# william-dawson/NTPoly

Hardware: AMD Instinct MI355X
Metric: TRS2 iters/s + SpGEMM nnz-out/s, N=262k ~200 nnz/row, 1/2/4/8 GPU (higher is better)
Workload: dtype f64

## Files before the change

### include/ntpoly_amd.h

```cpp
#ifndef NTPOLY_AMD_H
#define NTPOLY_AMD_H
#include "ntpoly_amd_process_grid.h"
#include "ntpoly_amd_psmatrix.h"
#include "ntpoly_amd_smatrix.h"
#include "ntpoly_amd_triplet_list.h"
#include "ntpoly_amd_permutation.h"
#include "ntpoly_amd_memory_pool.h"
#include "ntpoly_amd_solver_parameters.h"
#include "ntpoly_amd_density_matrix_solvers.h"
#include "ntpoly_amd_sign_solvers.h"
#include "ntpoly_amd_inverse_solvers.h"
#include "ntpoly_amd_square_root_solvers.h"
#include "ntpoly_amd_load_balancer.h"
#include "ntpoly_amd_eigen_bounds.h"
#include "ntpoly_amd_logging.h"
#include "ntpoly_amd_polynomial_solvers.h"
#include "ntpoly_amd_function_solvers.h"
#include "ntpoly_amd_linear_solvers.h"
#include "ntpoly_amd_eigen_solvers.h"
#include "ntpoly_amd_geometry.h"
#ifdef __cplusplus
extern "C" {
#endif

void ntpoly_amd_allreduce_max(double* values, const int* n);
int ntpoly_amd_band_order(const int* ih, int* newpos, long long* bandwidth);
void ntpoly_amd_band_scope_counts(long long* out);
void ntpoly_amd_band_searches(long long* out);
void ntpoly_amd_barrier();
void ntpoly_amd_block_algebra_counts(long long* out);
int ntpoly_amd_block_order(const int* ih, int* position);
int ntpoly_amd_block_order_of_pattern(const int* ih, int* position, int* ns);
void ntpoly_amd_block_scope_counts(long long* out);
void ntpoly_amd_column_fused_counts(long long* out);
int ntpoly_amd_comm_rank();
int ntpoly_amd_comm_size();
void ntpoly_amd_comm_split_matrix(const int* ih_this, int* ih_split, int* my_color, bool* split_slice);
void ntpoly_amd_complex_fusion_counts(long long* out);
int ntpoly_amd_device_count();
void ntpoly_amd_drop_block_caches();
void ntpoly_amd_exchange_stats(long long* out);
void ntpoly_amd_fill_prepartitioned(const int* ih_this, const int* ih_triplet_list);
void ntpoly_amd_finalize_comm();
void ntpoly_amd_fusion_counts(long long* out);
void ntpoly_amd_gather_matrix_to_process(const int* ih_this, int* ih_local, const int* within_slice_id);
int ntpoly_amd_get_option(const char* name);
void ntpoly_amd_get_spgemm_accum(long long* out, double* dout);
void ntpoly_amd_get_unique_id(char* out128);
void ntpoly_amd_grid_comm_info(const int* ih_grid, int* out);
void ntpoly_amd_halo_segment(const int* dim, const int* nranks, const int* s, const int* kmin, const int* kmax, int* a, int* b);
void ntpoly_amd_increment_identity(const int* ih_identity, int* ih_matB, const double* alpha);
void ntpoly_amd_init_comm(const char* id128, const int* rank, const int* nranks);
void ntpoly_amd_last_block_stats(long long* out, double* fill);
void ntpoly_amd_last_grouped_stats(long long* out, double* ratio);
void ntpoly_amd_last_spgemm_stats(long long* out, float* ms_numeric, float* ms_total);
int ntpoly_amd_last_spgemm_thin();
void ntpoly_amd_log_element_bool(const char* key, const int* nk, const bool* v);
void ntpoly_amd_log_element_int(const char* key, const int* nk, const int* v);
void ntpoly_amd_log_element_real(const char* key, const int* nk, const double* v);
void ntpoly_amd_log_element_string(const char* key, const int* nk, const char* v, const int* nv);
void ntpoly_amd_log_enter();
void ntpoly_amd_log_exit();
void ntpoly_amd_log_header(const char* text, const int* n);
void ntpoly_amd_log_list_element(const char* key, const int* nk);
void ntpoly_amd_malloc_stats(long long* calls, double* ms);
int ntpoly_amd_matrix_is_complex(const int* ih_this);
void ntpoly_amd_matrix_local_columns(const int* ih_this, int* c0, int* c1);
void ntpoly_amd_memory(long long* in_use, long long* cached);
int ntpoly_amd_norm_axpby(const int* ih_matA, const int* ih_matB, const double* alpha, const double* beta, double* norm);
void ntpoly_amd_panel_exchange_layout(const int* dim, const int* nranks, const int* me, const long long* req, const long long* cnt, int* sa, int* sb, long long* soff, int* ra, int* rb, long long* zoff);
void ntpoly_amd_panel_product_counts(long long* out);
void ntpoly_amd_panel_range(const int* dim, const int* nranks, const int* rank, int* c0, int* c1);
void ntpoly_amd_permutation_set(int* ih_this, const int* n, const int* index_lookup);
int ntpoly_amd_recurrence_step(const int* ih_P, const int* ih_Tkm2, int* ih_Tk, int* ih_R, const double* a, const double* c);
void ntpoly_amd_recurrence_step_count(long long* out);
void ntpoly_amd_release_cache();
void ntpoly_amd_reset_spgemm_accum();
void ntpoly_amd_session_begin(const int* complex_ok);
void ntpoly_amd_session_end();
void ntpoly_amd_set_option(const char* name, const int* value);
void ntpoly_amd_slab_algebra_counts(long long* out);
void ntpoly_amd_split_process_grid(const int* ih_old_grid, int* ih_new_grid, int* my_color, bool* split_slice);
void ntpoly_amd_square_root_order(const int* ih_Input, int* ih_Output, const int* ih_solver_parameters, const int* inverse, const int* order);
void ntpoly_amd_synchronize();
void ntpoly_amd_thin_slab_counts(long long* out);
void ntpoly_amd_tile2_counts(long long* out);
void ntpoly_amd_trace_get(double* value, double* energy, double* sigma, long long* nnz);
int ntpoly_amd_trace_iterations();
void ntpoly_amd_trace_times(double* setup_ms, double* loop_ms);
void ntpoly_amd_triplets_get(const int* ih_list, int* col, int* row, double* val);
void ntpoly_amd_triplets_set_c(int* ih_list, const long long* n, const int* col, const int* row, const double* val_ri);
void ntpoly_amd_triplets_set_r(int* ih_list, const long long* n, const int* col, const int* row, const double* val);
void ntpoly_amd_trs2_step(int* ih_X, int* ih_X2, const int* ih_WH, const double* trace, const double* threshold, double* energy_out, double* sigma_out, double* trace_io);

#ifdef __cplusplus
}
#endif
#endif
```

### ntpoly_amd/csrc/common.cpp

```cpp
#include <cstdio>
#include <cstdlib>
#include <chrono>
#include "common.hpp"

#include <cstring>
#include <mutex>

namespace ntp {

void fatal(const char* file, int line, const std::string& msg) {
  std::fprintf(stderr, "[ntpoly_amd] FATAL %s:%d: %s\n", file, line, msg.c_str());
  std::fflush(stderr);
  std::abort();
}

Context& ctx() {
  static Context* c = new Context();
  return *c;
}

void ensure_init() {
  Context& c = ctx();
  if (c.initialised) return;
  int ndev = 0;
  hipError_t e = hipGetDeviceCount(&ndev);
  if (e != hipSuccess || ndev == 0)
    NTP_FATAL("no HIP device visible: the ntpoly_amd engine has no CPU fallback");
  int local_rank = 0;
  if (const char* lr = std::getenv("LOCAL_RANK")) local_rank = std::atoi(lr);
  c.device = local_rank % ndev;
  HIP_CHECK(hipSetDevice(c.device));
  HIP_CHECK(hipStreamCreateWithFlags(&c.stream, hipStreamNonBlocking));
  HIP_CHECK(hipStreamCreateWithFlags(&c.comm_stream, hipStreamNonBlocking));
  hipDeviceProp_t prop;
  HIP_CHECK(hipGetDeviceProperties(&prop, c.device));
  c.num_cus = prop.multiProcessorCount;
  c.initialised = true;
}

long long& host_sync_count() {
  static long long n = 0;
  return n;
}
namespace {
struct SyncClock {
  bool on = std::getenv("NTPOLY_AMD_DEBUG_SYNC") != nullptr;
  long long calls = 0, slow = 0;
  double ms = 0.0;
  ~SyncClock() {
    if (on) std::fprintf(stderr, "[sync_stream] %lld waits, %.1f ms in them, %lld longer than 10 ms\n", calls, ms, slow);
  }
};
SyncClock& sync_clock() {
  static SyncClock c;
  return c;
}
}
void sync_stream() {
  host_sync_count() += 1;
  SyncClock& c = sync_clock();
  if (!c.on) {
    HIP_CHECK(hipStreamSynchronize(ctx().stream));
    return;
  }
  const auto t0 = std::chrono::steady_clock::now();
  HIP_CHECK(hipStreamSynchronize(ctx().stream));
  const double ms = std::chrono::duration<double, std::milli>(std::chrono::steady_clock::now() - t0).count();
  c.calls += 1;
  c.ms += ms;
  c.slow += ms > 10.0 ? 1 : 0;
}

namespace {
struct Pool {
  std::mutex mu;
  std::map<size_t, std::vector<void*>> free_lists;
  std::map<void*, size_t> live;
  std::map<const void*, unsigned long long> serial_of;
  unsigned long long next_serial = 1;
  size_t in_use = 0, cached = 0;
  long long n_malloc = 0;
  double ms_malloc = 0.0;
};
Pool& pool() {
  static Pool* p = new Pool();
  return *p;
}
size_t bucket(size_t bytes) {
  if (bytes < 512) return 512;
  const size_t big = (size_t)64 << 20;
  if (bytes > big) {
    const size_t want = bytes + bytes / 8;
    size_t p2 = big;
    while (p2 * 2 <= want) p2 <<= 1;
    const size_t step = p2 / 4;
    return (want + step - 1) / step * step;
  }
  size_t b = 512;
  while (b < bytes) b <<= 1;
  return b;
}
}

void* dev_alloc(size_t bytes) {
  ensure_init();
  const size_t b = bucket(bytes);
  Pool& P = pool();
  std::lock_guard<std::mutex> g(P.mu);
  auto it = P.free_lists.find(b);
  void* p = nullptr;
  size_t got = b;
  if (it == P.free_lists.end() || it->second.empty()) {
    it = P.free_lists.end();
    if (b >= ((size_t)1 << 20))
      for (auto jt = P.free_lists.upper_bound(b); jt != P.free_lists.end() && jt->first <= 2 * b; ++jt)
        if (!jt->second.empty()) { it = jt; got = jt->first; break; }
  }
  if (it != P.free_lists.end() && !it->second.empty()) {
    p = it->second.back();
    it->second.pop_back();
    P.cached -= got;
  } else {
    const auto t0 = std::chrono::steady_clock::now();
    hipError_t e = hipMalloc(&p, b);
    if (e != hipSuccess) {
      (void)hipGetLastError();
      for (auto& kv : P.free_lists) {
        for (void* q : kv.second) (void)hipFree(q);
        kv.second.clear();
      }
      P.cached = 0;
      HIP_CHECK(hipMalloc(&p, b));
    }
    P.n_malloc += 1;
    const double ms = std::chrono::duration<double, std::milli>(std::chrono::steady_clock::now() - t0).count();
    P.ms_malloc += ms;
    static const bool dbg = std::getenv("NTPOLY_AMD_DEBUG_ALLOC") != nullptr;
    if (dbg)
      std::fprintf(stderr, "[dev_alloc] hipMalloc %.1f MB (asked %.1f MB) took %.1f ms%s; in use %.1f GB, cached %.1f GB\n", b / 1048576.0,
                   bytes / 1048576.0, ms, e != hipSuccess ? " AFTER releasing the cache (out of memory)" : "", P.in_use / 1073741824.0,
                   P.cached / 1073741824.0);
  }
  P.live[p] = got;
  P.serial_of[p] = P.next_serial++;
  P.in_use += got;
  return p;
}

void dev_free(void* p) {
  if (!p) return;
  Pool& P = pool();
  std::lock_guard<std::mutex> g(P.mu);
  auto it = P.live.find(p);
// ... 96 lines not shown
```

### ntpoly_amd/csrc/common.hpp

```cpp
#pragma once
#include <hip/hip_runtime.h>

#include <cstdint>
#include <cstdio>
#include <cstdlib>
#include <map>
#include <string>
#include <utility>
#include <memory>
#include <vector>

namespace ntp {

[[noreturn]] void fatal(const char* file, int line, const std::string& msg);
#define NTP_FATAL(msg) ::ntp::fatal(__FILE__, __LINE__, (msg))
#define HIP_CHECK(expr)                                                              \
  do {                                                                               \
    hipError_t e_ = (expr);                                                          \
    if (e_ != hipSuccess)                                                            \
      ::ntp::fatal(__FILE__, __LINE__, std::string(#expr) + ": " + hipGetErrorString(e_)); \
  } while (0)

struct Context {
  int device = 0;
  hipStream_t stream = nullptr;
  hipStream_t comm_stream = nullptr;
  int num_cus = 256;
  bool initialised = false;
};
Context& ctx();
void ensure_init();
inline hipStream_t stream() { return ctx().stream; }
void sync_stream();
long long& host_sync_count();

struct ScalarFetch {
  const void* src[16];
  int words[16];
  void* dst[16];
  int n = 0;
  void add(const void* dev, int words8, void* host_dst) {
    src[n] = dev; words[n] = words8; dst[n] = host_dst; ++n;
  }
  void run();
};

void* dev_alloc(size_t bytes);
void dev_free(void* p);
unsigned long long dev_alloc_serial(const void* p);
void dev_release_cache();
size_t dev_bytes_in_use();
size_t dev_bytes_cached();
void dev_malloc_stats(long long* calls, double* ms);

template <typename T>
struct DevBuf {
  T* p = nullptr;
  size_t n = 0;
  DevBuf() = default;
  explicit DevBuf(size_t count) { alloc(count); }
  DevBuf(const DevBuf&) = delete;
  DevBuf& operator=(const DevBuf&) = delete;
  DevBuf(DevBuf&& o) noexcept : p(o.p), n(o.n) { o.p = nullptr; o.n = 0; }
  DevBuf& operator=(DevBuf&& o) noexcept {
    if (this != &o) {
      release();
      p = o.p; n = o.n; o.p = nullptr; o.n = 0;
    }
    return *this;
  }
  ~DevBuf() { release(); }
  void alloc(size_t count) {
    release();
    n = count;
    p = static_cast<T*>(dev_alloc((count ? count : 1) * sizeof(T)));
  }
  void release() {
    if (p) dev_free(p);
    p = nullptr; n = 0;
  }
  void upload(const T* host, size_t count) {
    if (count) HIP_CHECK(hipMemcpyAsync(p, host, count * sizeof(T), hipMemcpyHostToDevice, stream()));
  }
  void download(T* host, size_t count) const {
    const size_t bytes = count * sizeof(T);
    if (bytes > 0 && bytes <= 1024 && bytes % 8 == 0) {
      ScalarFetch f;
      f.add(p, (int)(bytes / 8), host);
      f.run();
      return;
    }
    if (count) HIP_CHECK(hipMemcpyAsync(host, p, bytes, hipMemcpyDeviceToHost, stream()));
    sync_stream();
  }
  void zero() { if (n) HIP_CHECK(hipMemsetAsync(p, 0, n * sizeof(T), stream())); }
};

constexpr size_t kIndexSlack = 1024;

struct SlabPlan {
  DevBuf<int32_t> blk_lo, blk_w, blk_kmin, blk_kn;
  DevBuf<int64_t> blk_toff;
  int64_t total = 0;
  int max_w = 0, max_kn = 0;
  int align = 0;
};
struct SlabForm {
  DevBuf<int32_t> first, last, count;
  DevBuf<int64_t> off;
  DevBuf<int64_t> tile_off;
  DevBuf<double> val, tiles;
  int64_t slots = 0;
  bool no_tile2 = false;
  std::unique_ptr<SlabPlan> next_plan;
  std::shared_ptr<struct DevMat> origin;
  mutable int64_t span_sum = -1;
  int row_pad = 1;
  DevBuf<int32_t> lab, plast;
  bool labelled() const { return lab.p != nullptr; }
};

struct DevMat {
  int32_t rows = 0, cols = 0;
  bool cplx = false;
  int64_t nnz = 0;
  DevBuf<int64_t> outer;
  DevBuf<int32_t> inner;
  DevBuf<double> val;
  DevBuf<int32_t> cnt;
  int64_t slots = 0;
  bool loose() const { return cnt.p != nullptr; }
  mutable int zero_free = 0;
  std::unique_ptr<SlabForm> slab;
  bool expanded() const { return slab != nullptr; }
  std::shared_ptr<struct BlockForm> blk;
  bool blocked() const { return blk != nullptr; }
  mutable int block_hint = 0;
  mutable int slab_hint = 0;

  DevMat() = default;
  DevMat(int32_t r, int32_t c, bool z) { reset_empty(r, c, z); }
  DevMat(DevMat&&) noexcept = default;
  DevMat& operator=(DevMat&&) noexcept = default;
  void reset_empty(int32_t r, int32_t c, bool z);
  void alloc(int32_t r, int32_t c, bool z, int64_t nz);
  DevMat clone() const;
  size_t wval() const { return cplx ? 2 : 1; }
};

DevMat packed_copy(const DevMat& M);

struct HostTriplets {
  std::vector<int32_t> col, row;
  std::vector<double> val;
  bool cplx = false;
  size_t size() const { return col.size(); }
};

}
```

### ntpoly_amd/csrc/kernels.hip

```cpp
#include "kernels.hpp"
#include "device_util.hpp"
#include "spgemm_grouped.hpp"
#include "slab_types.hpp"
#include "spgemm_tile.hpp"
#include "spgemm_block.hpp"

#include <hip/hip_runtime.h>

#include <algorithm>
#include <cstdlib>
#include <climits>
#include <cmath>
#include <cstring>
#include <type_traits>
#include <numeric>
#include <utility>

#include <rocprim/device/device_radix_sort.hpp>

namespace ntp {

namespace {

__global__ __launch_bounds__(1024) void k_scan_excl_i64(const int64_t* __restrict__ in,
// ... 533 lines not shown
        }
      }
      if (!more) break;
      s_cur = s_nxt;
      use_a = !use_a;
    }
    asm volatile("s_waitcnt vmcnt(0)" ::: "memory");
    kv0 = nk0; kv1 = nk1;
    bv0 = nb0; bv1 = nb1;
  }
  __builtin_amdgcn_wave_barrier();

#pragma unroll
  for (int r = 0; r < 2; ++r) {
    const bool act = r == 0 ? act0 : act1;
    if (!act) continue;
    const int j = r == 0 ? j0 : j1;
    const int lo = r == 0 ? lo0 : lo1, span = r == 0 ? span0 : span1;
    const double* acc = r == 0 ? acc0 : acc1;
    const int64_t base = tmpoff[j];
    int cnt = 0;
    for (int s0 = 0; s0 < span; s0 += WAVE) {
      const int s = s0 + lane;
      const double v = (s < span) ? acc[s] : 0.0;
      const double sv = __dmul_rn(alpha, v);
      const bool keep = (s < span) && ((dense_rule & 1) ? (fabs(v) > threshold) : (fabs(sv) > threshold));
      const unsigned long long m = __ballot(keep);
      if (keep) {
        const int64_t pos = base + cnt + __popcll(m & lanemask_lt());
        out_inner[pos] = lo + s;
        out_val[pos] = sv;
      }
      cnt += __popcll(m);
    }
    if (lane == 0) count[j] = cnt;
  }
}

template <typename T>
__global__ __launch_bounds__(256) void k_slab_expand_a(Csc A, const int32_t* __restrict__ afirst,
                                                       const int64_t* __restrict__ aeoff, T* __restrict__ aexp) {
  const int k = (blockIdx.x * blockDim.x + threadIdx.x) / WAVE;
  if (k >= A.cols) return;
  const int lane = lane_id();
  const int64_t s = A.outer[k], e = A.outer[k + 1];
  if (e <= s) return;
  const T* __restrict__ Av = static_cast<const T*>(A.val);
  T* __restrict__ dst = aexp + aeoff[k] - afirst[k];
  for (int64_t p = s + lane; p < e; p += WAVE) {
    const int r = A.inner[p];
    const int prev = (p > s) ? A.inner[p - 1] : r - 1;
    dst[r] = Av[p];
    for (int h = prev + 1; h < r; ++h) dst[h] = Sc<T>::zero();
  }
}

__global__ void k_span_aligned(const int32_t* __restrict__ cmin, const int32_t* __restrict__ cmax, int32_t* __restrict__ span, int n, int al) {
  const int k = blockIdx.x * blockDim.x + threadIdx.x;
  if (k >= n) return;
  const int f = cmin[k], l = cmax[k];
  span[k] = l >= f ? (l / al + 1) * al - f / al * al : 0;
}
template <typename T>
__global__ __launch_bounds__(256) void k_aligned_offsets(const int32_t* __restrict__ cmin, const int32_t* __restrict__ cmax,
                                                         int64_t* __restrict__ off, T* __restrict__ exp, int n, int al) {
  const int k = (blockIdx.x * blockDim.x + threadIdx.x) / WAVE;
  if (k >= n) return;
  const int lane = lane_id();
  const int f = cmin[k], l = cmax[k];
  if (l < f) return;
  const int64_t slot = off[k];
  const int head = f - f / al * al, tail = (l / al + 1) * al - 1 - l;
  for (int i = lane; i < head; i += WAVE) exp[slot + i] = Sc<T>::zero();
  for (int i = lane; i < tail; i += WAVE) exp[slot + head + (l - f + 1) + i] = Sc<T>::zero();
  if (lane == 0) off[k] = slot + head;
}

template <int J>
__global__ __launch_bounds__(256) void k_slab_plan(int ncols, const int32_t* __restrict__ bfirst,
                                                   const int32_t* __restrict__ blast, const int32_t* __restrict__ cmin,
                                                   const int32_t* __restrict__ cmax, int32_t* __restrict__ blk_lo,
                                                   int32_t* __restrict__ blk_w, int32_t* __restrict__ blk_kmin,
                                                   int32_t* __restrict__ blk_kn, int64_t* __restrict__ bsz,
                                                   int64_t* __restrict__ tsz, int nblocks, int align16 = 0) {
  const int b = (blockIdx.x * blockDim.x + threadIdx.x) / WAVE;
  const int lane = lane_id();
  if (b < nblocks) {
    const int j = b * J + lane;
    const bool has = lane < J && j < ncols && blast[min(j, ncols - 1)] >= 0;
    const int kmin = wave_min_i32(has ? bfirst[j] : INT_MAX), kmax = wave_max_i32(has ? blast[j] : -1);
    if (kmax >= kmin && kmax - kmin >= 4096) {
      if (lane == 0) {
        blk_lo[b] = 0;
        blk_w[b] = 1 << 30;
        blk_kmin[b] = kmin;
        blk_kn[b] = kmax - kmin + 1;
        bsz[b] = 0;
        tsz[b] = 0;
      }
    } else {
      int lo = INT_MAX, hi = -1;
      for (int k = (kmax >= kmin) ? kmin + lane : 0; k <= kmax; k += WAVE) {
        const int c0 = cmin[k], c1 = cmax[k];
        if (c1 >= c0) {
          lo = min(lo, c0);
          hi = max(hi, c1 + 1);
        }
      }
      lo = wave_min_i32(lo);
      hi = wave_max_i32(hi);
      if (lane == 0) {
        if (align16 > 0 && hi > lo) {
          lo = lo / align16 * align16;
          hi = (hi + align16 - 1) / align16 * align16;
        }
        const int w = (hi > lo) ? hi - lo : 0;
        const int kn = (w > 0 && kmax >= kmin) ? kmax - kmin + 1 : 0;
        blk_lo[b] = w > 0 ? lo : 0;
        blk_w[b] = w;
        blk_kmin[b] = kn > 0 ? kmin : 0;
        blk_kn[b] = kn;
        bsz[b] = (int64_t)((kn + 1) & ~1) * J;
        tsz[b] = (int64_t)w * J;
      }
    }
  }
}

constexpr int kOffParts = 64;
__global__ __launch_bounds__(256) void k_slab_offsets(const int32_t* __restrict__ blk_w, const int32_t* __restrict__ blk_kn,
                                                      const int64_t* __restrict__ tsz, const int64_t* __restrict__ bsz,
                                                      int nblocks, int part, int64_t* __restrict__ toff,
                                                      int64_t* __restrict__ boff, unsigned long long* __restrict__ stats) {
  __shared__ long long wsum[2][4];
  __shared__ int wmax[2][4];
  const int lane = lane_id(), wave = threadIdx.x / WAVE;
  const int p0 = blockIdx.x * part, p1 = min(nblocks, p0 + part);
  if (p0 >= nblocks) return;
  auto block_sum = [&](long long& a, long long& b) {
    a = wave_sum_i64(a);
    b = wave_sum_i64(b);
    __syncthreads();
    if (lane == 0) { wsum[0][wave] = a; wsum[1][wave] = b; }
    __syncthreads();
    a = wsum[0][0] + wsum[0][1] + wsum[0][2] + wsum[0][3];
    b = wsum[1][0] + wsum[1][1] + wsum[1][2] + wsum[1][3];
  };
  long long carry_t = 0, carry_b = 0;
  {
    int i = threadIdx.x;
    for (; i + 7 * 256 < p0; i += 8 * 256) {
      long long t[8], u[8];
#pragma unroll
      for (int e = 0; e < 8; ++e) {
        t[e] = tsz[i + e * 256];
        u[e] = boff ? (long long)bsz[i + e * 256] : 0;
      }
#pragma unroll
      for (int e = 0; e < 8; ++e) { carry_t += t[e]; carry_b += u[e]; }
    }
    for (; i < p0; i += 256) {
      carry_t += tsz[i];
      if (boff) carry_b += bsz[i];
    }
  }
  block_sum(carry_t, carry_b);
  int mw = 0, mk = 0;
  for (int base = p0; base < p1; base += 256) {
    const int i = base + threadIdx.x;
    const long long t = i < p1 ? (long long)tsz[i] : 0, b = (boff && i < p1) ? (long long)bsz[i] : 0;
    if (i < p1) {
      mw = max(mw, blk_w[i]);
      mk = max(mk, blk_kn[i]);
    }
    long long xt = t, xb = b;
    for (int o = 1; o < WAVE; o <<= 1) {
      const long long at = __shfl_up(xt, o, WAVE), ab = __shfl_up(xb, o, WAVE);
      if (lane >= o) { xt += at; xb += ab; }
    }
    __syncthreads();
    if (lane == WAVE - 1) { wsum[0][wave] = xt; wsum[1][wave] = xb; }
    __syncthreads();
    long long pt = carry_t + xt - t, pb = carry_b + xb - b;
    for (int q = 0; q < wave; ++q) { pt += wsum[0][q]; pb += wsum[1][q]; }
    if (i < p1) {
      toff[i] = pt;
      if (boff) boff[i] = pb;
    }
    carry_t += wsum[0][0] + wsum[0][1] + wsum[0][2] + wsum[0][3];
    carry_b += wsum[1][0] + wsum[1][1] + wsum[1][2] + wsum[1][3];
  }
  if (p1 == nblocks && threadIdx.x == 0) {
    toff[nblocks] = carry_t;
    if (boff) boff[nblocks] = carry_b;
  }
  mw = wave_max_i32(mw);
  mk = wave_max_i32(mk);
  __syncthreads();
  if (lane == 0) { wmax[0][wave] = mw; wmax[1][wave] = mk; }
  __syncthreads();
  if (threadIdx.x == 0 && stats) {
    atomicMax(&stats[16], (unsigned long long)max(max(wmax[0][0], wmax[0][1]), max(wmax[0][2], wmax[0][3])));
    atomicMax(&stats[17], (unsigned long long)max(max(wmax[1][0], wmax[1][1]), max(wmax[1][2], wmax[1][3])));
  }
}

template <typename T, int J>
__global__ __launch_bounds__(256) void k_slab_expand_b(Csc B, const int32_t* __restrict__ blk_kmin,
                                                       const int32_t* __restrict__ blk_kn,
                                                       const int64_t* __restrict__ blk_boff, T* __restrict__ bblk,
                                                       int nblocks, int pitch, int fuse_a,
                                                       const int64_t* __restrict__ aeoff, T* __restrict__ aexp,
                                                       const int32_t* __restrict__ clen,
                                                       int64_t* __restrict__ blk_prod) {
  extern __shared__ __attribute__((aligned(16))) char smem[];
  T* tile = reinterpret_cast<T*>(smem);
  const int b = xcd_block(nblocks);
  if (b < 0) return;
  const int kn = blk_kn[b], kmin = blk_kmin[b];
  if (kn == 0 && !fuse_a) return;
  const bool tiled = kn > 0;
  const T* __restrict__ Bv = static_cast<const T*>(B.val);
  const int wave = threadIdx.x / WAVE, lane = lane_id();
  constexpr int CH = 5, NCOL = J / 4;
  int idx[NCOL][CH];
  T val[NCOL][CH];
#pragma unroll
  for (int q = 0; q < NCOL; ++q) {
    const int j = min(b * J + wave + 4 * q, B.cols - 1);
    const int64_t s = B.outer[j];
#pragma unroll
    for (int c = 0; c < CH; ++c) {
      idx[q][c] = B.inner[s + c * WAVE + lane];
      val[q][c] = Bv[s + c * WAVE + lane];
    }
  }
  const int kne = (kn + 1) & ~1;
  for (int jj = 0; jj < J; ++jj)
    for (int i = threadIdx.x; i < kne; i += blockDim.x) tile[jj * pitch + i] = Sc<T>::zero();
  __syncthreads();
  long long nprod = 0;
#pragma unroll
  for (int q = 0; q < NCOL; ++q) {
    const int jj = wave + 4 * q;
    const int j = b * J + jj;
    if (j >= B.cols) break;
    const int64_t s = B.outer[j], e = col_end(B, j);
    if (e <= s) continue;
    const int first = readlane_i32(idx[q][0], 0);
    T* __restrict__ dst = fuse_a ? aexp + aeoff[j] - first : nullptr;
    int carry = first - 1;
#pragma unroll
    for (int c = 0; c < CH; ++c) {
      const int64_t p = s + c * WAVE + lane;
      const int r = idx[q][c];
      int prev = __shfl_up(r, 1, WAVE);
      if (lane == 0) prev = carry;
      if (p < e) {
        if (clen) nprod += clen[r];
        if (tiled) tile[jj * pitch + (r - kmin)] = val[q][c];
        if (fuse_a) {
          dst[r] = val[q][c];
          for (int h = prev + 1; h < r; ++h) dst[h] = Sc<T>::zero();
        }
      }
      carry = readlane_i32(r, WAVE - 1);
    }
    for (int64_t p = s + CH * WAVE + lane; p < e; p += WAVE) {
      const int r = B.inner[p];
      const T v = Bv[p];
      if (clen) nprod += clen[r];
      if (tiled) tile[jj * pitch + (r - kmin)] = v;
      if (fuse_a) {
        const int prev = B.inner[p - 1];
        dst[r] = v;
        for (int h = prev + 1; h < r; ++h) dst[h] = Sc<T>::zero();
      }
    }
  }
  nprod = wave_sum_i64(nprod);
  __shared__ long long sprod[4];
  if (lane == 0) sprod[wave] = nprod;
  __syncthreads();
  if (threadIdx.x == 0) blk_prod[b] = sprod[0] + sprod[1] + sprod[2] + sprod[3];
  T* __restrict__ out = bblk + blk_boff[b];
  const int total = kne * J;
// ... 1548 lines not shown
__global__ void k_remap_gather(const unsigned long long* __restrict__ keys, const unsigned int* __restrict__ payload,
                               int64_t nkeep, const T* __restrict__ val, int32_t* __restrict__ inner_out,
                               T* __restrict__ val_out, int32_t* __restrict__ colcount) {
  const int64_t p = (int64_t)blockIdx.x * blockDim.x + threadIdx.x;
  const bool live = p < nkeep;
  const unsigned long long k = live ? keys[p] : ~0ull;
  if (live) {
    inner_out[p] = (int32_t)(k & 0xffffffffull);
    val_out[p] = val[payload[p]];
  }
  const int col = (int)(k >> 32), lane = lane_id();
  const int prev = __shfl_up(col, 1, WAVE);
  const bool leader = live && (lane == 0 || col != prev);
  const unsigned long long heads = __ballot(leader), alive = __ballot(live);
  if (leader) {
    const unsigned long long later = heads & ~((2ull << lane) - 1ull);
    const int end = later ? __builtin_ctzll(later) : (int)__popcll(alive);
    atomicAdd(&colcount[col], end - lane);
  }
}
__global__ void k_count_valid(const unsigned long long* __restrict__ keys, int64_t n,
                              unsigned long long* __restrict__ out) {
  __shared__ unsigned long long sc[4];
  unsigned long long c = 0;
  for (int64_t p = (int64_t)blockIdx.x * blockDim.x + threadIdx.x; p < n; p += (int64_t)gridDim.x * blockDim.x)
    c += keys[p] != ~0ull ? 1ull : 0ull;
  c = (unsigned long long)wave_sum_i64((int64_t)c);
  if (lane_id() == 0) sc[threadIdx.x / WAVE] = c;
  __syncthreads();
  if (threadIdx.x == 0) atomicAdd(out, sc[0] + sc[1] + sc[2] + sc[3]);
}

__global__ void k_shift_outer(const int64_t* __restrict__ in, int64_t* __restrict__ out, int n, int64_t shift) {
  const int j = blockIdx.x * blockDim.x + threadIdx.x;
  if (j <= n) out[j] = in[j] + shift;
}

__global__ void k_rebase_i64(const int64_t* __restrict__ in, int64_t* __restrict__ out, int n, int64_t add) {
  const int i = blockIdx.x * blockDim.x + threadIdx.x;
  if (i < n) out[i] = in[i] - in[0] + add;
}
__global__ void k_linear_i64(int64_t* __restrict__ out, int64_t n, int64_t step) {
  const int64_t i = (int64_t)blockIdx.x * blockDim.x + threadIdx.x;
  if (i < n) out[i] = i * step;
}
__global__ void k_fill_i64(int64_t* __restrict__ out, int64_t n, int64_t v) {
  const int64_t i = (int64_t)blockIdx.x * blockDim.x + threadIdx.x;
  if (i < n) out[i] = v;
}
__global__ void k_row_range(Csc A, int* __restrict__ mm) {
  const int j = blockIdx.x * blockDim.x + threadIdx.x;
  int lo = INT_MAX, hi = -1;
  if (j < A.cols) {
    const int64_t s = A.outer[j], e = A.outer[j + 1];
    if (e > s) {
      lo = A.inner[s];
      hi = A.inner[e - 1];
    }
  }
  lo = wave_min_i32(lo);
  hi = wave_max_i32(hi);
  if (lane_id() == 0) {
    if (lo != INT_MAX) atomicMin(&mm[0], lo);
    if (hi >= 0) atomicMax(&mm[1], hi);
  }
}

}

EngineOptions& options() {
  static EngineOptions* o = [] {
    auto* e = new EngineOptions();
    if (const char* v = std::getenv("NTPOLY_AMD_HALO_OVERLAP")) e->halo_overlap = std::atoi(v);
    if (const char* v = std::getenv("NTPOLY_AMD_SPGEMM_FMA")) e->spgemm_fma = std::atoi(v);
    if (const char* v = std::getenv("NTPOLY_AMD_ARITHMETIC")) {
      const std::string a(v);
      if (a == "fma") e->spgemm_fma = 1;
      else if (a == "unfused") e->spgemm_fma = 0;
      else NTP_FATAL("NTPOLY_AMD_ARITHMETIC must be fma or unfused, not " + a);
    }
    if (const char* v = std::getenv("NTPOLY_AMD_TILE_ROWS")) e->tile_rows = std::atoi(v);
    if (const char* v = std::getenv("NTPOLY_AMD_TILE_WAVES")) e->tile_waves = std::atoi(v);
    if (const char* v = std::getenv("NTPOLY_AMD_PLAN_AHEAD")) e->plan_ahead = std::atoi(v);
    if (const char* v = std::getenv("NTPOLY_AMD_SLAB_ALGEBRA")) e->slab_algebra = std::atoi(v);
    if (const char* v = std::getenv("NTPOLY_AMD_PANEL_SESSIONS")) e->panel_sessions = std::atoi(v);
    if (const char* v = std::getenv("NTPOLY_AMD_COMPLEX_PANELS")) e->complex_panels = std::atoi(v);
    if (const char* v = std::getenv("NTPOLY_AMD_THIN_SLAB_COMPLEX")) e->thin_slab_complex = std::atoi(v);
    if (const char* v = std::getenv("NTPOLY_AMD_COMPLEX_POLY_SESSIONS")) e->complex_poly_sessions = std::atoi(v);
    if (const char* v = std::getenv("NTPOLY_AMD_COMPLEX_DENSITY")) e->complex_density = std::atoi(v);
    if (const char* v = std::getenv("NTPOLY_AMD_BLOCK_SCOPE_COMPLEX")) e->block_scope_complex = std::atoi(v);
    if (const char* v = std::getenv("NTPOLY_AMD_BLOCK_UNFUSED")) e->block_unfused = std::atoi(v);
    return e;
  }();
  return *o;
}
SpgemmStats& last_spgemm_stats() {
  static SpgemmStats* s = new SpgemmStats();
  return *s;
}
SpgemmAccum& spgemm_accum() {
  static SpgemmAccum* a = new SpgemmAccum();
  return *a;
}

namespace {
template <typename TIn>
void scan_async(const TIn* d_in, int64_t* d_out, int64_t n) {
  if (n <= 4096) {
    if constexpr (sizeof(TIn) == 8) hipLaunchKernelGGL(k_scan_excl_i64, dim3(1), dim3(1024), 0, stream(), (const int64_t*)d_in, d_out, n);
    else hipLaunchKernelGGL(k_scan_excl_i32, dim3(1), dim3(1024), 0, stream(), (const int32_t*)d_in, d_out, n);
    return;
  }
  const int nb = (int)((n + 2047) / 2048);
  DevBuf<int64_t> sums((size_t)nb), offs((size_t)nb + 1);
  hipLaunchKernelGGL((k_scan_block_sums<TIn>), dim3(nb), dim3(256), 0, stream(), d_in, n, sums.p);
  hipLaunchKernelGGL(k_scan_excl_i64, dim3(1), dim3(1024), 0, stream(), sums.p, offs.p, (int64_t)nb);
  hipLaunchKernelGGL((k_scan_block_apply<TIn>), dim3(nb), dim3(256), 0, stream(), d_in, n, offs.p, d_out);
}
void reduce_sum2_async(const double* part, int n, double* out_dev) {
  if (n <= 8192) {
    hipLaunchKernelGGL(k_reduce_sum2, dim3(1), dim3(256), 0, stream(), part, n, out_dev, n);
    return;
  }
  const int chunk = 2048, g = (n + chunk - 1) / chunk;
  DevBuf<double> lvl((size_t)2 * g);
  hipLaunchKernelGGL(k_reduce_sum2, dim3(g), dim3(256), 0, stream(), part, n, lvl.p, chunk);
  hipLaunchKernelGGL(k_reduce_sum2, dim3(1), dim3(256), 0, stream(), lvl.p, g, out_dev, g);
}
}

constexpr int FT_BLOCKS = 64;
__global__ __launch_bounds__(256) void k_fused_totals(const int32_t* __restrict__ count, int n, const long long* __restrict__ a,
                                                      const long long* __restrict__ b, const double* __restrict__ part,
                                                      int m, const double* __restrict__ lvl_in, double* __restrict__ out,
                                                      int stage) {
  __shared__ long long si[3][4];
  __shared__ double sd[2][4];
  const int wave = threadIdx.x / WAVE, lane = lane_id();
  long long c = 0, x = 0, y = 0;
  double d = 0.0, t = 0.0;
  if (stage == 0) {
    const int g = blockIdx.x;
    const int n0 = (int)((int64_t)n * g / FT_BLOCKS), n1 = (int)((int64_t)n * (g + 1) / FT_BLOCKS);
#pragma unroll 8
    for (int i = n0 + threadIdx.x; i < n1; i += 256) c += count[i];
    const int m0 = (int)((int64_t)m * g / FT_BLOCKS), m1 = (int)((int64_t)m * (g + 1) / FT_BLOCKS);
#pragma unroll 2
    for (int i = m0 + threadIdx.x; i < m1; i += 256) {
      x += a[i];
      if (b) y += b[i];
      d = __dadd_rn(d, part[2 * i]);
      t = __dadd_rn(t, part[2 * i + 1]);
    }
  } else {
    const long long* li = reinterpret_cast<const long long*>(lvl_in);
    for (int g = threadIdx.x; g < FT_BLOCKS; g += 256) {
      c += li[5 * g]; x += li[5 * g + 1]; y += li[5 * g + 2];
      d = __dadd_rn(d, lvl_in[5 * g + 3]);
      t = __dadd_rn(t, lvl_in[5 * g + 4]);
    }
  }
  c = wave_sum_i64(c); x = wave_sum_i64(x); y = wave_sum_i64(y);
  d = wave_sum_f64(d); t = wave_sum_f64(t);
  if (lane == 0) { si[0][wave] = c; si[1][wave] = x; si[2][wave] = y; sd[0][wave] = d; sd[1][wave] = t; }
  __syncthreads();
  if (threadIdx.x == 0) {
    long long* oi = reinterpret_cast<long long*>(out) + (stage == 0 ? 5 * blockIdx.x : 0);
    double* od = out + (stage == 0 ? 5 * blockIdx.x : 0);
    for (int q = 0; q < 3; ++q) oi[q] = si[q][0] + si[q][1] + si[q][2] + si[q][3];
    od[3] = __dadd_rn(__dadd_rn(sd[0][0], sd[0][1]), __dadd_rn(sd[0][2], sd[0][3]));
    od[4] = __dadd_rn(__dadd_rn(sd[1][0], sd[1][1]), __dadd_rn(sd[1][2], sd[1][3]));
  }
}

void scan_i32_async(const int32_t* d_in, int64_t* d_out, int64_t n) { scan_async<int32_t>(d_in, d_out, n); }
void scan_i64_async(const int64_t* d_in, int64_t* d_out, int64_t n) { scan_async<int64_t>(d_in, d_out, n); }

namespace {
struct FetchArgs {
  const unsigned long long* src[16];
  int words[16];
  int n;
};
__global__ __launch_bounds__(64) void k_fetch(FetchArgs a, unsigned long long* __restrict__ host_mapped) {
  int off = 0;
  for (int s = 0; s < a.n; ++s) {
    for (int i = threadIdx.x; i < a.words[s]; i += 64) host_mapped[off + i] = a.src[s][i];
    off += a.words[s];
  }
  __threadfence_system();
}
}

void ScalarFetch::run() {
  static unsigned long long* host = nullptr;
  static unsigned long long* dev = nullptr;
  constexpr int kMaxWords = 512;
  if (!host) {
    HIP_CHECK(hipHostMalloc(reinterpret_cast<void**>(&host), kMaxWords * 8, hipHostMallocMapped));
    HIP_CHECK(hipHostGetDevicePointer(reinterpret_cast<void**>(&dev), host, 0));
  }
  FetchArgs a;
  a.n = n;
  int total = 0;
  for (int s = 0; s < n; ++s) {
    a.src[s] = static_cast<const unsigned long long*>(src[s]);
    a.words[s] = words[s];
    total += words[s];
  }
  if (total > kMaxWords) NTP_FATAL("ScalarFetch: too many words");
  if (total) hipLaunchKernelGGL(k_fetch, dim3(1), dim3(64), 0, stream(), a, dev);
  sync_stream();
  int off = 0;
  for (int s = 0; s < n; ++s) {
    std::memcpy(dst[s], host + off, (size_t)words[s] * 8);
    off += words[s];
  }
  n = 0;
}

static int64_t exclusive_scan_i64_from_i32(const int32_t* d_in, int64_t* d_out, int64_t n) {
  scan_async<int32_t>(d_in, d_out, n);
  int64_t total = 0;
  ScalarFetch f;
  f.add(d_out + n, 1, &total);
  f.run();
  return total;
}
int64_t exclusive_scan_i64(const int64_t* d_in, int64_t* d_out, int64_t n) {
  scan_async<int64_t>(d_in, d_out, n);
  int64_t total = 0;
  HIP_CHECK(hipMemcpyAsync(&total, d_out + n, sizeof(int64_t), hipMemcpyDeviceToHost, stream()));
  sync_stream();
  return total;
}

namespace {
struct TimedCall {
  hipEvent_t ev[4];
};
std::vector<hipEvent_t>& event_pool() {
  static auto* p = new std::vector<hipEvent_t>();
  return *p;
}
std::vector<TimedCall>& pending_timings() {
  static auto* p = new std::vector<TimedCall>();
  return *p;
}
hipEvent_t get_event() {
  auto& pool = event_pool();
  if (!pool.empty()) {
    hipEvent_t e = pool.back();
    pool.pop_back();
    return e;
// ... 30 lines not shown
  unsigned long long serial = 0, epoch = 0;
  int64_t nnz = -1;
  int32_t cols = 0;
  DevBuf<int32_t> dmin, dmax;
  DevBuf<int64_t> doff;
  DevBuf<double> dexp;
  int64_t max_tile = 0;
  int align = 1;
};
__global__ __launch_bounds__(256) void k_count_zero_values(Csc A, unsigned long long* __restrict__ out) {
  const int j = (blockIdx.x * blockDim.x + threadIdx.x) / WAVE;
  if (j >= A.cols) return;
  const int lane = lane_id();
  const double* __restrict__ v = static_cast<const double*>(A.val);
  int c = 0;
  for (int64_t p = A.outer[j] + lane, e = col_end(A, j); p < e; p += WAVE) c += v[p] == 0.0 ? 1 : 0;
  const unsigned long long m = __ballot(c != 0);
  if (m && lane == 0) atomicAdd(out, 1ull);
}
__global__ void k_span_block_max(const int32_t* __restrict__ span, int n, int J, unsigned long long* __restrict__ out) {
  const int b = blockIdx.x * blockDim.x + threadIdx.x;
  if (b * J >= n) return;
  unsigned long long t = 0;
  for (int j = b * J; j < min(n, (b + 1) * J); ++j) t += (unsigned long long)span[j];
  atomicMax(out, t);
}
DotOperand*& dot_operand_slot() {
  static DotOperand* c = new DotOperand();
  return c;
}
void drop_dot_operand() { *dot_operand_slot() = DotOperand(); }
const DotOperand& dot_operand(const DevMat& D) {
  DotOperand* c = dot_operand_slot();
  const unsigned long long ser = dev_alloc_serial(D.val.p);
  const int want_al = options().spgemm_fma == 1 ? tile_expand_align() : 1;
  if (c->val == D.val.p && c->serial == ser && ser != 0 && c->epoch == value_epoch() && c->nnz == D.nnz && c->cols == D.cols &&
      c->align == want_al)
    return *c;
  const int n = D.cols;
  c->dmin.alloc((size_t)n); c->dmax.alloc((size_t)n); c->doff.alloc((size_t)n + 1);
  DevBuf<int32_t> dlen((size_t)n), dspan((size_t)n);
  hipLaunchKernelGGL(k_col_extent, dim3(cdiv(n, 256)), dim3(256), 0, stream(), view(D), c->dmin.p, c->dmax.p, dlen.p);
  const int al = options().spgemm_fma == 1 ? tile_expand_align() : 1;
  if (al > 1) hipLaunchKernelGGL(k_span_aligned, dim3(cdiv(n, 256)), dim3(256), 0, stream(), c->dmin.p, c->dmax.p, dspan.p, n, al);
  else hipLaunchKernelGGL(k_span_of, dim3(cdiv(n, 256)), dim3(256), 0, stream(), c->dmin.p, c->dmax.p, dspan.p, n);
  scan_async<int32_t>(dspan.p, c->doff.p, (int64_t)n);
  DevBuf<unsigned long long> tmax(1);
  tmax.zero();
  hipLaunchKernelGGL(k_span_block_max, dim3(cdiv(cdiv(n, SLAB_J), 256)), dim3(256), 0, stream(), dspan.p, n, SLAB_J, tmax.p);
  int64_t total = 0;
  unsigned long long hmax = 0;
  {
    ScalarFetch f;
    f.add(c->doff.p + n, 1, &total);
    f.add(tmax.p, 1, &hmax);
    f.run();
  }
  c->max_tile = (int64_t)hmax;
  c->dexp.alloc((size_t)total + 1);
  if (al > 1)
    hipLaunchKernelGGL(k_aligned_offsets<double>, dim3(cdiv((int64_t)n * WAVE, 256)), dim3(256), 0, stream(), c->dmin.p, c->dmax.p,
                       c->doff.p, c->dexp.p, n, al);
  c->align = al;
  hipLaunchKernelGGL(k_slab_expand_a<double>, dim3(cdiv((int64_t)n * WAVE, 256)), dim3(256), 0, stream(), view(D), c->dmin.p,
                     c->doff.p, c->dexp.p);
  c->val = D.val.p;
  c->serial = ser;
  c->epoch = value_epoch();
  c->nnz = D.nnz;
  c->cols = n;
  return *c;
}
}

long long* fusion_counts() {
  static long long c[3] = {0, 0, 0};
  return c;
}
long long* complex_fusion_counts() {
  static long long c[3] = {0, 0, 0};
  return c;
}
long long* tile2_counts() {
  static long long c[2] = {0, 0};
  return c;
}

void flush_spgemm_timers() {
  auto& pend = pending_timings();
  if (pend.empty()) return;
  SpgemmAccum& acc = spgemm_accum();
  for (size_t i = 0; i < pend.size(); ++i) {
    float t_all = 0.f, t_num = 0.f;
    HIP_CHECK(hipEventSynchronize(pend[i].ev[1]));
    HIP_CHECK(hipEventElapsedTime(&t_all, pend[i].ev[0], pend[i].ev[1]));
    HIP_CHECK(hipEventElapsedTime(&t_num, pend[i].ev[2], pend[i].ev[3]));
    acc.ms_total += t_all;
    acc.ms_numeric += t_num;
    if (i + 1 == pend.size()) {
      last_spgemm_stats().ms_total = t_all;
      last_spgemm_stats().ms_numeric = t_num;
    }
    for (int k = 0; k < 4; ++k) event_pool().push_back(pend[i].ev[k]);
  }
  pend.clear();
}

namespace {
__global__ __launch_bounds__(256) void k_pack_slab(int ncols, const int32_t* __restrict__ first, const int32_t* __restrict__ last,
                                                   const int64_t* __restrict__ off, const double* __restrict__ val,
                                                   const int64_t* __restrict__ outer, int32_t* __restrict__ inner,
                                                   double* __restrict__ out) {
  const int j = (blockIdx.x * blockDim.x + threadIdx.x) / WAVE;
  if (j >= ncols) return;
  const int lane = lane_id();
  const int f = first[j], l = last[j];
  int64_t pos = outer[j];
  const double* __restrict__ src = val + off[j];
  for (int r0 = f; r0 <= l; r0 += WAVE) {
    const int r = r0 + lane;
    const double v = r <= l ? src[r - f] : 0.0;
    const unsigned long long m = __ballot(v != 0.0);
    if (v != 0.0) {
      const int64_t q = pos + __popcll(m & lanemask_lt());
      inner[q] = r;
      out[q] = v;
    }
    pos += __popcll(m);
  }
}
__global__ __launch_bounds__(256) void k_pack_slab_c(int ncols, const int32_t* __restrict__ first, const int32_t* __restrict__ last,
                                                     const int64_t* __restrict__ off, const double2* __restrict__ val,
                                                     const int64_t* __restrict__ outer, int32_t* __restrict__ inner,
                                                     double2* __restrict__ out) {
  const int j = (blockIdx.x * blockDim.x + threadIdx.x) / WAVE;
  if (j >= ncols) return;
  const int lane = lane_id();
  const int f = first[j], l = last[j];
  int64_t pos = outer[j];
  const double2* __restrict__ src = val + off[j];
  for (int r0 = f; r0 <= l; r0 += WAVE) {
    const int r = r0 + lane;
    const double2 v = r <= l ? src[r - f] : make_double2(0.0, 0.0);
    const bool nz = v.x != 0.0 || v.y != 0.0;
    const unsigned long long m = __ballot(nz);
    if (nz) {
      const int64_t q = pos + __popcll(m & lanemask_lt());
      inner[q] = r;
      out[q] = v;
    }
    pos += __popcll(m);
  }
}
template <int MAXCH, int NW>
void launch_pair3(int bin_lo, int bin_hi, int wrt, const DevMat& A, const DevMat& B, const int32_t* lo, const int32_t* span,
                  const uint8_t* binarr, const int64_t* tmpoff, int32_t* out_inner, double* out_val, int32_t* count,
                  double alpha, double thr, int dense_rule) {
  const int ngroups = cdiv(B.cols, 2);
  const int nblocks = cdiv(ngroups, NW);
  const size_t lds = (size_t)NW * 2 * (size_t)wrt * sizeof(double);
  hipLaunchKernelGGL((k_spgemm_pair3<MAXCH, NW>), dim3(xcd_grid(nblocks)), dim3(NW * WAVE), lds, stream(), view(A), view(B),
                     lo, span, binarr, bin_lo, bin_hi, tmpoff, out_inner, out_val, count, alpha, thr, dense_rule, nblocks, wrt);
}

template <typename T, int W, int NW>
void launch_window(int bin, const DevMat& A, const DevMat& B, const int32_t* lo, const int32_t* span,
// ... 1059 lines not shown

namespace {
__global__ void k_pack_reduce4(const double* __restrict__ tot, const int* __restrict__ flag, double* __restrict__ out) {
  out[0] = tot[3];
  out[1] = 0.0;
  out[2] = tot[4];
  out[3] = flag[0] == 0 ? 1.0 : 0.0;
}
__global__ void k_slab_runs_addr(const int32_t* __restrict__ first, const int32_t* __restrict__ last,
                                 const unsigned long long* __restrict__ addr, unsigned long long fallback,
                                 SlabRun* __restrict__ runs, int n, int elem_bytes) {
  const int k = blockIdx.x * blockDim.x + threadIdx.x;
  if (k >= n + 4) return;
  const bool any = k < n && last[k] >= first[k];
  SlabRun r;
  const unsigned long long a = any ? addr[k] : fallback;
  r.addr_lo = (uint32_t)a;
  r.addr_hi = (uint32_t)(a >> 32) & 0xffffu;
  r.nbytes = any ? (uint32_t)(last[k] - first[k] + 1) * (uint32_t)elem_bytes : 0u;
  r.flags = kBufferFlags;
  r.first = any ? first[k] : (1 << 30);
  r.first8 = any ? first[k] * elem_bytes : 0;
  r.span62 = any ? (last[k] - first[k] + 1) + 62 : 0;
  r.pad = 0;
  runs[k] = r;
}

__global__ __launch_bounds__(256) void k_slab_order_steps(const int32_t* __restrict__ lab, const int32_t* __restrict__ blk_kmin,
                                                          const int32_t* __restrict__ blk_kn, const int64_t* __restrict__ tile_off,
                                                          const double* __restrict__ tiles_in, const SlabRun* __restrict__ runs,
                                                          int ncols, double* __restrict__ tiles_out, SlabRun* __restrict__ blkruns,
                                                          int32_t* __restrict__ steps, int nblocks) {
  extern __shared__ unsigned long long sk[];
  const int b = xcd_block(nblocks);
  if (b < 0) return;
  const int kn = blk_kn[b], kmin = blk_kmin[b];
  if (kn == 0) return;
  int m = 1;
  while (m < kn) m <<= 1;
  for (int i = threadIdx.x; i < m; i += blockDim.x)
    sk[i] = i < kn ? (((unsigned long long)(unsigned)lab[kmin + i] << 32) | (unsigned)i) : ~0ull;
  __syncthreads();
  for (int k = 2; k <= m; k <<= 1) {
    for (int j = k >> 1; j > 0; j >>= 1) {
      for (int i = threadIdx.x; i < m; i += blockDim.x) {
        const int l = i ^ j;
        if (l > i) {
          const bool up = (i & k) == 0;
          const unsigned long long x = sk[i], y = sk[l];
          if ((x > y) == up) { sk[i] = y; sk[l] = x; }
        }
      }
      __syncthreads();
    }
  }
  const int64_t toff = tile_off[b];
  const int64_t rbase = toff / SLAB_J + 4 * (int64_t)b;
  for (int t = threadIdx.x; t < kn + 4; t += blockDim.x) {
    if (t < kn) {
      const int i = (int)(unsigned)(sk[t] & 0xffffffffull);
      const int k = kmin + i;
      if (steps) steps[rbase + t] = k;
      SlabRun r = runs[k];
      r.pad = i * (int)(SLAB_J * sizeof(double));
      blkruns[rbase + t] = r;
    } else {
      if (steps) steps[rbase + t] = ncols;
      blkruns[rbase + t] = runs[ncols];
    }
  }
  if (!tiles_out) return;
  const double2* __restrict__ src = reinterpret_cast<const double2*>(tiles_in + toff);
  double2* __restrict__ dst = reinterpret_cast<double2*>(tiles_out + toff);
  for (int i = threadIdx.x; i < kn * (SLAB_J / 2); i += blockDim.x) {
    const int t = i / (SLAB_J / 2), q = i % (SLAB_J / 2);
    dst[(size_t)t * (SLAB_J / 2) + q] = src[(size_t)(unsigned)(sk[t] & 0xffffffffull) * (SLAB_J / 2) + q];
  }
}
}

namespace {
template <int J = SLAB_J>
void launch_slab_plan(SlabPlan& P, int n, const int32_t* first, const int32_t* last, const int32_t* afirst, const int32_t* alast,
                      int align, unsigned long long* stats, DevBuf<int64_t>* tile_offsets = nullptr) {
  const int snb = cdiv(n, J);
  P.blk_lo.alloc(snb); P.blk_w.alloc(snb); P.blk_kmin.alloc(snb); P.blk_kn.alloc(snb);
  P.blk_toff.alloc((size_t)snb + 1);
  P.align = align;
  DevBuf<int64_t> bsz(snb), tsz(snb);
  if (tile_offsets) tile_offsets->alloc((size_t)snb + 1);
  hipLaunchKernelGGL((k_slab_plan<J>), dim3(cdiv((int64_t)snb * WAVE, 256)), dim3(256), 0, stream(), n, first, last, afirst,
                     alast, P.blk_lo.p, P.blk_w.p, P.blk_kmin.p, P.blk_kn.p, bsz.p, tsz.p, snb, align);
  if (options().plan_fused != 0) {
    const int part = cdiv(cdiv(snb, kOffParts), 256) * 256;
    hipLaunchKernelGGL(k_slab_offsets, dim3(cdiv(snb, part)), dim3(256), 0, stream(), P.blk_w.p, P.blk_kn.p, tsz.p, bsz.p, snb, part,
                       P.blk_toff.p, tile_offsets ? tile_offsets->p : (int64_t*)nullptr, stats);
    return;
  }
  hipLaunchKernelGGL(k_slab_reduce, dim3(64), dim3(256), 0, stream(), P.blk_w.p, P.blk_kn.p, snb, (const int32_t*)nullptr, 0, stats);
  scan_async<int64_t>(tsz.p, P.blk_toff.p, (int64_t)snb);
  if (tile_offsets) scan_async<int64_t>(bsz.p, tile_offsets->p, (int64_t)snb);
}
}

bool slab_step(DevMat& X, SlabFusion& fu, double threshold, bool dense_rule, const SlabHalo* halo) {
  fu.done = false;
  if (!X.expanded() || X.cplx || (!halo && X.rows != X.cols) || !fu.D || fu.D->cplx || fu.D->loose() || fu.D->expanded() ||
      fu.D->rows != X.rows || fu.D->cols != X.cols || (fu.mode != 1 && fu.mode != 2))
    return false;
  const bool tile = options().spgemm_fma == 1;
  if ((options().spgemm_variant >= 0 && !(tile && options().spgemm_variant / 100 == 6)) || (options().spgemm_fma && !tile) || options().spgemm_force_bin > 0 || !options().fused_update)
    return false;
  const SlabForm& in = *X.slab;
  int trows = 1;
  if (tile) {
    trows = tile_rows();
    while (trows > 1 && (in.row_pad % (16 * trows) != 0 || (halo && halo->row_pad % (16 * trows) != 0))) trows >>= 1;
  }
  const int n = X.cols, snb = cdiv(n, SLAB_J);
  const DotOperand& dop = dot_operand(*fu.D);
  if (!tile && dop.max_tile > SLAB_DTILE) return false;
  const bool timing = options().time_kernels != 0;
  EventTimer t_all(timing), t_num(timing);
  t_all.start();
  SpgemmStats st;
  st.nnz_a = st.nnz_b = X.nnz;
  DevBuf<int32_t> count((size_t)n), ofirst((size_t)n), olast((size_t)n);
  DevBuf<int64_t> tmpoff((size_t)n + 1);
  DevBuf<int64_t> zwords((size_t)4 * snb + 4 + 48);
  zwords.zero();
  if (!tile) count.zero();
  int64_t* fz_flag = zwords.p;
  int64_t* fz_pnnz = zwords.p + 2;
  double* fz_part = reinterpret_cast<double*>(zwords.p + 3 + 2 * (size_t)snb);
  unsigned long long* stats = reinterpret_cast<unsigned long long*>(zwords.p + 4 * (size_t)snb + 4);
  unsigned long long* next_stats = stats + 24;
  const int ka = halo ? halo->ka : 0, nka = halo ? halo->kb - halo->ka : n;
  const int plan_align = tile ? 16 * tile_rows() : 0;
  SlabPlan own_plan;
  SlabPlan* plan = &own_plan;
  if (!halo && in.next_plan && in.next_plan->align == plan_align && (int64_t)in.next_plan->blk_lo.n == snb) {
    plan = in.next_plan.get();
  } else if (halo && halo->plan && halo->plan->align == plan_align && (int64_t)halo->plan->blk_lo.n == snb) {
    plan = halo->plan;
  } else {
    const int32_t* afirst = halo ? halo->first - ka : in.first.p;
    const int32_t* alast = halo ? halo->last - ka : in.last.p;
    launch_slab_plan(own_plan, n, in.first.p, in.last.p, afirst, alast, plan_align, stats);
    unsigned long long hs[3] = {0, 0, 0};
    ScalarFetch f;
    f.add(own_plan.blk_toff.p + snb, 1, &own_plan.total);
    f.add(stats + 16, 3, hs);
    f.run();
    own_plan.max_w = (int)hs[0];
    own_plan.max_kn = (int)hs[1];
  }
  DevBuf<int32_t>&blk_lo = plan->blk_lo, &blk_w = plan->blk_w, &blk_kmin = plan->blk_kmin, &blk_kn = plan->blk_kn;
  DevBuf<int64_t>& blk_toff = plan->blk_toff;
  const int64_t tmp_total = plan->total;
  const unsigned long long hst[2] = {(unsigned long long)plan->max_w, (unsigned long long)plan->max_kn};
  const int64_t max_w = (int64_t)hst[0];
  auto give_up = [&]() {
    if (timing) {
      event_pool().push_back(t_all.a); event_pool().push_back(t_all.b);
      event_pool().push_back(t_num.a); event_pool().push_back(t_num.b);
    }
    return false;
  };
  if (max_w <= 0 || (!tile && max_w > 8 * SLAB_SL * WAVE)) return give_up();
  if (tile && !spgemm_tile_fits((int)hst[1], (int)max_w)) return give_up();
  if (in.labelled() && (int64_t)hst[1] > 2048) return give_up();
  if (!tile)
    hipLaunchKernelGGL((k_slab_tmpoff<SLAB_J>), dim3(cdiv(n + 1, 256)), dim3(256), 0, stream(), n, blk_w.p, blk_toff.p, tmpoff.p);
  DevBuf<char> runs(((size_t)nka + 4) * sizeof(SlabRun));
  if (halo)
    hipLaunchKernelGGL(k_slab_runs_addr, dim3(cdiv(nka + 4, 256)), dim3(256), 0, stream(), halo->first, halo->last, halo->addr,
                       (unsigned long long)reinterpret_cast<uintptr_t>(in.val.p), reinterpret_cast<SlabRun*>(runs.p), nka, 8);
  else
    hipLaunchKernelGGL(k_slab_runs, dim3(cdiv(n + 4, 256)), dim3(256), 0, stream(), in.first.p, in.last.p, in.off.p,
                       reinterpret_cast<const char*>(in.val.p), 8, reinterpret_cast<SlabRun*>(runs.p), n);
  const size_t oslots = (size_t)tmp_total + (size_t)tmp_total / 5 + kIndexSlack;
  const bool runs_only = tile && !halo && options().tile_runs_only != 0;
  DevBuf<double> oval(oslots), otiles(runs_only ? 0 : oslots);
  SlabFuseArgs fz;
  fz.am = fu.am; fz.bm = fu.bm; fz.thr_m = fu.threshold;
  fz.xexp = in.val.p; fz.xoff = in.off.p; fz.xmin = in.first.p; fz.xmax = in.last.p;
  fz.dexp = dop.dexp.p; fz.doff = dop.doff.p; fz.dmin = dop.dmin.p; fz.dmax = dop.dmax.p;
  fz.ofirst = ofirst.p; fz.olast = olast.p; fz.tiles = runs_only ? nullptr : otiles.p;
  fz.part = fz_part; fz.pnnz = reinterpret_cast<long long*>(fz_pnnz); fz.flag = reinterpret_cast<int*>(fz_flag);
  fz.col_offset = fu.col_offset;
  int64_t* blk_prod = zwords.p + 3 + snb;
  const bool labelled = in.labelled() && !halo && !tile;
  if (in.labelled() && halo) return give_up();
  DevBuf<double> tiles_ord;
  DevBuf<char> blkruns;
  DevBuf<int32_t> steps, oplast;
  const bool rowoff = labelled && options().label_rowoff != 0;
  if (labelled) {
    const size_t nrec = in.tiles.n / SLAB_J + 4 * (size_t)snb + 8;
    blkruns.alloc(nrec * sizeof(SlabRun));
    oplast.alloc((size_t)n);
    if (!rowoff) {
      tiles_ord.alloc(in.tiles.n);
      steps.alloc(nrec);
    }
    int m = 1;
    while (m < (int)hst[1]) m <<= 1;
    hipLaunchKernelGGL(k_slab_order_steps, dim3(xcd_grid(snb)), dim3(256), (size_t)m * 8, stream(), in.lab.p, blk_kmin.p, blk_kn.p,
                       in.tile_off.p, in.tiles.p, reinterpret_cast<const SlabRun*>(runs.p), n, tiles_ord.p,
                       reinterpret_cast<SlabRun*>(blkruns.p), steps.p, snb);
    fz.lab = in.lab.p;
    fz.blkruns = reinterpret_cast<const SlabRun*>(blkruns.p);
    fz.steps = steps.p;
    fz.xplast = in.plast.p;
    fz.oplast = oplast.p;
  }
  const bool scope_lab = tile && halo && !in.labelled() && scope_labels() != nullptr && in.plast.p != nullptr && fu.mode != 0;
  const bool tile_labelled = tile && ((in.labelled() && !halo) || scope_lab);
  if (tile_labelled) {
    oplast.alloc((size_t)n);
    fz.lab = scope_lab ? scope_labels() : in.lab.p;
    fz.xplast = in.plast.p;
    fz.oplast = oplast.p;
  }
  fz.prod = reinterpret_cast<long long*>(blk_prod);
  if (!halo || halo->count) fz.in_count = halo ? halo->count - ka : in.count.p;
  DevBuf<char> fz_args;
  if (!tile) {
    fz_args.alloc(sizeof(SlabFuseArgs));
    fz_args.upload(reinterpret_cast<const char*>(&fz), sizeof(SlabFuseArgs));
  }
  const int dr = dense_rule ? 1 : 0;
  t_num.start();
  auto launch = [&](auto nw_tag, auto mode_tag, auto epi_tag) {
    constexpr int FNW = decltype(nw_tag)::value;
    hipLaunchKernelGGL((k_spgemm_slab<SLAB_J, SLAB_SL, FNW, decltype(mode_tag)::value, decltype(epi_tag)::value>),
                       dim3(xcd_grid(snb)), dim3(FNW * WAVE), 0, stream(), reinterpret_cast<const SlabRun*>(runs.p) - ka,
                       (labelled && !rowoff) ? tiles_ord.p : in.tiles.p, in.tile_off.p, blk_kmin.p, blk_kn.p, blk_lo.p, blk_w.p, blk_toff.p, (int32_t*)nullptr,
                       oval.p, count.p, 1.0, threshold, dr, n, snb, reinterpret_cast<const SlabFuseArgs*>(fz_args.p));
  };
  auto by_mode = [&](auto nw_tag, auto mode_tag) {
    if (fu.mode == 1) launch(nw_tag, mode_tag, std::integral_constant<int, 1>{});
    else launch(nw_tag, mode_tag, std::integral_constant<int, 2>{});
  };
  DevBuf<int64_t> tile_ooff, tile_otoff;
  bool used_tile2 = false;
  if (tile) {
    tile_ooff.alloc((size_t)n + 1);
    tile_otoff.alloc((size_t)snb + 1);
    TileLaunch tl;
    tl.runs = reinterpret_cast<const SlabRun*>(runs.p) - ka;
    tl.bblk = in.tiles.p; tl.blk_boff = in.tile_off.p;
    if (in.tiles.p == nullptr || in.tile_off.p == nullptr) {
      tl.bblk = nullptr; tl.blk_boff = nullptr;
      tl.brun_first = in.first.p; tl.brun_last = in.last.p; tl.brun_off = in.off.p; tl.brun_val = in.val.p; tl.bbytes = in.val.n * sizeof(double); tl.brun_pad = in.row_pad;
    }
    tl.blk_kmin = blk_kmin.p; tl.blk_kn = blk_kn.p; tl.blk_lo = blk_lo.p;
    tl.blk_w = blk_w.p; tl.blk_toff = blk_toff.p; tl.out_val = oval.p; tl.count = count.p;
    tl.ofirst = ofirst.p; tl.olast = olast.p; tl.ooff = tile_ooff.p; tl.otoff = tile_otoff.p;
    tl.alpha = 1.0; tl.threshold = threshold; tl.dense_rule = dr; tl.ncols = n; tl.nblocks = snb;
    tl.max_kn = (int)hst[1]; tl.max_w = (int)max_w; tl.epi = fu.mode; tl.fz = &fz; tl.rows = trows; tl.labelled = tile_labelled;
    tl.nrows = X.rows;
    if (!halo) {
      tl.abase = in.val.p; tl.abytes = in.val.n * sizeof(double);
      tl.dbase = dop.dexp.p; tl.dbytes = dop.dexp.n * sizeof(double);
    }
    if (!halo && options().tile2 != 0 && !in.no_tile2) used_tile2 = launch_spgemm_tile2(tl, reinterpret_cast<int*>(fz_flag) + 2);
    if (!used_tile2) launch_spgemm_tile(tl);
  } else if (rowoff) {
    if (max_w > 6 * SLAB_SL * WAVE) by_mode(std::integral_constant<int, 8>{}, std::integral_constant<int, 9>{});
    else if (max_w > SLAB_NW * SLAB_SL * WAVE) by_mode(std::integral_constant<int, 6>{}, std::integral_constant<int, 9>{});
    else by_mode(std::integral_constant<int, SLAB_NW>{}, std::integral_constant<int, 9>{});
  } else if (max_w > 6 * SLAB_SL * WAVE) by_mode(std::integral_constant<int, 8>{}, std::integral_constant<int, 0>{});
  else if (max_w > SLAB_NW * SLAB_SL * WAVE) by_mode(std::integral_constant<int, 6>{}, std::integral_constant<int, 0>{});
  else by_mode(std::integral_constant<int, SLAB_NW>{}, std::integral_constant<int, 8>{});
  t_num.stop();
  DevBuf<double> lvl((size_t)5 * FT_BLOCKS), tot(5);
  hipLaunchKernelGGL(k_fused_totals, dim3(FT_BLOCKS), dim3(256), 0, stream(), count.p, n,
                     reinterpret_cast<const long long*>(fz_pnnz), reinterpret_cast<const long long*>(blk_prod), fz_part, snb,
                     (const double*)nullptr, lvl.p, 0);
  hipLaunchKernelGGL(k_fused_totals, dim3(1), dim3(256), 0, stream(), (const int32_t*)nullptr, 0, (const long long*)nullptr,
                     (const long long*)nullptr, (const double*)nullptr, 0, lvl.p, tot.p, 1);
  unsigned long long raw[5] = {0, 0, 0, 0, 0};
  int64_t flagv[2] = {0, 0};
  DevBuf<double> red4;
  if (halo && halo->reduce) {
    red4.alloc(4);
    hipLaunchKernelGGL(k_pack_reduce4, dim3(1), dim3(1), 0, stream(), tot.p, reinterpret_cast<const int*>(fz_flag), red4.p);
    halo->reduce->allreduce(red4.p);
  }
  std::unique_ptr<SlabPlan> next;
  unsigned long long next_hs[3] = {0, 0, 0};
  if (tile && !halo && options().plan_ahead != 0) {
    next.reset(new SlabPlan());
    launch_slab_plan(*next, n, ofirst.p, olast.p, ofirst.p, olast.p, plan_align, next_stats);
  }
  DevMat R;
  R.rows = X.rows;
  R.cols = n;
  R.cplx = false;
  R.zero_free = 1;
  R.slab.reset(new SlabForm());
  R.slab->first = std::move(ofirst);
  R.slab->last = std::move(olast);
  R.slab->count = std::move(count);
  R.slab->row_pad = tile ? 16 * trows : 1;
  R.slab->no_tile2 = in.no_tile2;
  R.slab->off = tile ? std::move(tile_ooff) : std::move(tmpoff);
  if (tile) R.slab->tile_off = std::move(tile_otoff);
  R.slab->val = std::move(oval);
  if (runs_only) { R.slab->tile_off.release(); } else R.slab->tiles = std::move(otiles);
  R.slab->slots = tmp_total;
  {
    ScalarFetch f;
    f.add(tot.p, 5, raw);
    f.add(fz_flag, 2, flagv);
    if (red4.p) f.add(red4.p, 4, halo->reduce->reduced);
    if (next) {
      f.add(next->blk_toff.p + snb, 1, &next->total);
      f.add(next_stats + 16, 3, next_hs);
    }
    if (halo && halo->before_fetch) halo->before_fetch(R, reinterpret_cast<const long long*>(tot.p), f);
    f.run();
    if (red4.p) halo->reduce->done = true;
  }
  t_all.stop();
  if (next) {
    next->max_w = (int)next_hs[0];
    next->max_kn = (int)next_hs[1];
  }
  if (std::getenv("NTPOLY_AMD_DEBUG_SPGEMM"))
    std::fprintf(stderr, "[slab_step] mode %d slots %lld w %llu kn %llu in-slots %lld nnz-in %lld plan %s\n", fu.mode, (long long)tmp_total,
                 hst[0], hst[1], (long long)in.slots, (long long)X.nnz, plan == &own_plan ? "made here" : "left by the step before");
  if (timing) {
    if (pending_timings().size() >= 4096) flush_spgemm_timers();
    pending_timings().push_back(TimedCall{{t_all.a, t_all.b, t_num.a, t_num.b}});
  }
  if (used_tile2 && (int32_t)flagv[1] != 0) {
    X.slab->no_tile2 = true;
    tile2_counts()[1] += 1;
    return slab_step(X, fu, threshold, dense_rule, halo);
  }
  if (used_tile2) tile2_counts()[0] += 1;
  if ((int32_t)flagv[0] != 0) {
    fu.refused += 1;
    fusion_counts()[2] += 1;
    return false;
  }
  const int64_t nnz = (int64_t)raw[0], pnz = (int64_t)raw[1];
  double hd[2];
  std::memcpy(hd, &raw[3], 2 * sizeof(double));
  const int64_t nnz_in = X.nnz;
  R.nnz = nnz;
  R.slab->next_plan = std::move(next);
  if (!tile) R.slab->tile_off = std::move(plan->blk_toff);
  if (labelled || tile_labelled) {
    R.slab->lab = std::move(X.slab->lab);
    R.slab->plast = std::move(oplast);
  }
  if (halo) fu.result = std::move(R);
  else X = std::move(R);
  fu.done = true;
  fu.dot = hd[0];
  fu.trace = hd[1];
  fu.product_nnz = pnz;
  fusion_counts()[fu.mode == 1 ? 0 : 1] += 1;
  st.slab = 1;
  st.fused = fu.mode;
  st.nnz_c = pnz;
  st.tmp_entries = tmp_total;
  const bool counted = !halo || halo->count;
  st.products = counted ? (int64_t)raw[2] : -1;
  last_spgemm_stats() = st;
  SpgemmAccum& acc = spgemm_accum();
  acc.calls += 1;
  if (counted) acc.products += (int64_t)raw[2];
  acc.nnz_c += pnz;
  acc.alg_bytes += 12.0 * (double)(2 * nnz_in + pnz) + 4.0 * (3.0 * n + 3);
  return true;
}

bool slab_from_csc(DevMat& Xs, DevBuf<int32_t>& lab) {
  if (Xs.cplx || Xs.loose() || Xs.expanded() || Xs.rows != Xs.cols || Xs.nnz == 0) return false;
  const int n = Xs.cols, snb = cdiv(n, SLAB_J);
  std::unique_ptr<SlabForm> f(new SlabForm());
  f->first.alloc((size_t)n); f->last.alloc((size_t)n); f->count.alloc((size_t)n); f->off.alloc((size_t)n + 1);
  f->tile_off.alloc((size_t)snb + 1); f->plast.alloc((size_t)n);
  DevBuf<int32_t> span((size_t)n), blk_lo(snb), blk_w(snb), blk_kmin(snb), blk_kn(snb);
  DevBuf<int64_t> bsz(snb), tsz(snb), dummy(snb);
  DevBuf<unsigned long long> stats(24);
  stats.zero();
  hipLaunchKernelGGL(k_col_extent, dim3(cdiv(n, 256)), dim3(256), 0, stream(), view(Xs), f->first.p, f->last.p, f->count.p);
  const int al = options().spgemm_fma == 1 ? tile_expand_align() : 1;
  if (al > 1) hipLaunchKernelGGL(k_span_aligned, dim3(cdiv(n, 256)), dim3(256), 0, stream(), f->first.p, f->last.p, span.p, n, al);
  else hipLaunchKernelGGL(k_span_of, dim3(cdiv(n, 256)), dim3(256), 0, stream(), f->first.p, f->last.p, span.p, n);
  scan_async<int32_t>(span.p, f->off.p, (int64_t)n);
  hipLaunchKernelGGL((k_slab_plan<SLAB_J>), dim3(cdiv((int64_t)snb * WAVE, 256)), dim3(256), 0, stream(), n, f->first.p, f->last.p,
                     f->first.p, f->last.p, blk_lo.p, blk_w.p, blk_kmin.p, blk_kn.p, bsz.p, tsz.p, snb);
  hipLaunchKernelGGL(k_slab_reduce, dim3(64), dim3(256), 0, stream(), blk_w.p, blk_kn.p, snb, (const int32_t*)nullptr, 0, stats.p);
  scan_async<int64_t>(bsz.p, f->tile_off.p, (int64_t)snb);
  int64_t tot_val = 0, tot_tiles = 0;
  unsigned long long hst[2] = {0, 0};
  {
    ScalarFetch ft;
    ft.add(f->off.p + n, 1, &tot_val);
    ft.add(f->tile_off.p + snb, 1, &tot_tiles);
    ft.add(stats.p + 16, 2, hst);
    ft.run();
  }
  const int64_t max_w = (int64_t)hst[0], max_kn = (int64_t)hst[1];
  const int pitch = ((int)max_kn + 1) | 1;
  if (max_w <= 0 || max_w > 8 * SLAB_SL * WAVE || (size_t)pitch * SLAB_J * 8 > 128 * 1024) return false;
  if ((double)tot_val > 2.0 * (double)Xs.nnz + (al > 1 ? 2.0 * al * (double)n : 0.0)) return false;
  f->val.alloc((size_t)tot_val + kIndexSlack);
  if (al > 1)
    hipLaunchKernelGGL(k_aligned_offsets<double>, dim3(cdiv((int64_t)n * WAVE, 256)), dim3(256), 0, stream(), f->first.p, f->last.p,
                       f->off.p, f->val.p, n, al);
  f->row_pad = al;
  f->tiles.alloc((size_t)tot_tiles + 16 * SLAB_J + kIndexSlack);
  hipLaunchKernelGGL(k_slab_expand_a<double>, dim3(cdiv((int64_t)n * WAVE, 256)), dim3(256), 0, stream(), view(Xs), f->first.p,
                     f->off.p, f->val.p);
  if ((size_t)pitch * SLAB_J * 8 > 64 * 1024) {
    static bool raised = false;
    if (!raised) {
      HIP_CHECK(hipFuncSetAttribute(reinterpret_cast<const void*>(&k_slab_expand_b<double, SLAB_J>),
                                    hipFuncAttributeMaxDynamicSharedMemorySize, 144 * 1024));
      raised = true;
    }
  }
  hipLaunchKernelGGL((k_slab_expand_b<double, SLAB_J>), dim3(xcd_grid(snb)), dim3(256), (size_t)pitch * SLAB_J * 8, stream(), view(Xs),
                     blk_kmin.p, blk_kn.p, f->tile_off.p, f->tiles.p, snb, pitch, 0, (const int64_t*)nullptr, (double*)nullptr,
                     (const int32_t*)nullptr, dummy.p);
  hipLaunchKernelGGL(k_col_plast, dim3(cdiv((int64_t)n * WAVE, 256)), dim3(256), 0, stream(), view(Xs), lab.p, f->plast.p);
  f->slots = std::max(tot_val, tot_tiles);
  f->lab = std::move(lab);
  DevMat R;
  R.rows = Xs.rows;
// ... 1492 lines not shown
  fo->first.alloc((size_t)n); fo->last.alloc((size_t)n); fo->count.alloc((size_t)n); fo->off.alloc((size_t)n + 1);
  DevBuf<int32_t> span((size_t)n);
  DevBuf<int64_t> base((size_t)n + 1);
  DevBuf<unsigned long long> stat(2);
  stat.zero();
  hipLaunchKernelGGL(k_sa_span, dim3(cdiv(n, 256)), dim3(256), 0, stream(), fa.first.p, fa.last.p, have_b ? fb->first.p : nullptr,
                     have_b ? fb->last.p : nullptr, n, al, span.p);
  scan_async<int32_t>(span.p, base.p, (int64_t)n);
  fo->val.alloc(((size_t)bound + kIndexSlack) * (cplx ? 2 : 1));
  if (cplx) {
    const double2* va = reinterpret_cast<const double2*>(fa.val.p);
    const double2* vb = have_b ? reinterpret_cast<const double2*>(fb->val.p) : nullptr;
    double2* vo = reinterpret_cast<double2*>(fo->val.p);
    if (have_b)
      hipLaunchKernelGGL((k_sa_axpby<double2, true>), dim3(cdiv((int64_t)n * WAVE, 256)), dim3(256), 0, stream(), n, fa.first.p, fa.last.p, fa.off.p,
                         va, fb->first.p, fb->last.p, fb->off.p, vb, base.p, al, alpha, beta, thr, vo, fo->first.p, fo->last.p, fo->count.p,
                         fo->off.p, stat.p, bound);
    else
      hipLaunchKernelGGL((k_sa_axpby<double2, false>), dim3(cdiv((int64_t)n * WAVE, 256)), dim3(256), 0, stream(), n, fa.first.p, fa.last.p, fa.off.p,
                         va, (const int32_t*)nullptr, (const int32_t*)nullptr, (const int64_t*)nullptr, (const double2*)nullptr, base.p, al, 1.0, 0.0,
                         0.0, vo, fo->first.p, fo->last.p, fo->count.p, fo->off.p, stat.p, bound);
  } else if (have_b)
    hipLaunchKernelGGL((k_sa_axpby<double, true>), dim3(cdiv((int64_t)n * WAVE, 256)), dim3(256), 0, stream(), n, fa.first.p, fa.last.p, fa.off.p,
                       fa.val.p, fb->first.p, fb->last.p, fb->off.p, fb->val.p, base.p, al, alpha, beta, thr, fo->val.p, fo->first.p,
                       fo->last.p, fo->count.p, fo->off.p, stat.p, bound);
  else
    hipLaunchKernelGGL((k_sa_axpby<double, false>), dim3(cdiv((int64_t)n * WAVE, 256)), dim3(256), 0, stream(), n, fa.first.p, fa.last.p, fa.off.p,
                       fa.val.p, (const int32_t*)nullptr, (const int32_t*)nullptr, (const int64_t*)nullptr, (const double*)nullptr,
                       base.p, al, 1.0, 0.0, 0.0, fo->val.p, fo->first.p, fo->last.p, fo->count.p, fo->off.p, stat.p, bound);
  DevBuf<long long> tot;
  sa_sum_counts(fo->count.p, n, tot);
  int64_t nnz = 0, slots = 0;
  unsigned long long hs = 0;
  {
    ScalarFetch ft;
    ft.add(tot.p, 1, &nnz);
    ft.add(base.p + n, 1, &slots);
    ft.add(stat.p, 1, &hs);
    ft.run();
  }
  if (hs != 0) return false;
  fo->row_pad = al;
  fo->slots = slots;
  DevMat R;
  R.rows = X.rows; R.cols = n; R.cplx = cplx; R.nnz = nnz; R.zero_free = 1;
  R.slab = std::move(fo);
  Out = std::move(R);
  return true;
}

bool slab_axpby(const DevMat& A, DevMat& B, double alpha, double beta, double threshold) {
  if (!sa_operand(A) || !sa_operand(B) || A.cols != B.cols || &A == &B) return false;
  if (alpha == 0.0 || beta == 0.0) return false;
  if (A.zero_free != 1 || B.zero_free != 1) return false;
  DevMat R;
  if (!sa_axpby_impl(&A, B, R, alpha, beta, threshold)) return false;
  value_epoch() += 1;
  B = std::move(R);
  return true;
}

bool slab_axpby_to(const DevMat& A, const DevMat& B, DevMat& Out, double alpha, double beta, double threshold) {
  if (!sa_operand(A) || !sa_operand(B) || A.cols != B.cols || &A == &B) return false;
  if (alpha == 0.0 || beta == 0.0 || A.zero_free != 1 || B.zero_free != 1) return false;
  DevMat R;
  if (!sa_axpby_impl(&A, B, R, alpha, beta, threshold)) return false;
  Out = std::move(R);
  return true;
}

bool slab_clone(const DevMat& A, DevMat& Out) {
  if (!sa_operand(A) || A.zero_free != 1) return false;
  return sa_axpby_impl(nullptr, A, Out, 1.0, 0.0, 0.0);
}

bool slab_scale(DevMat& A, double c) {
  if (!sa_operand(A) || c == 0.0 || A.slab->origin) return false;
  value_epoch() += 1;
  SlabForm& f = *A.slab;
  hipLaunchKernelGGL(k_sa_scale<double>, dim3(cdiv((int64_t)A.cols * WAVE, 256)), dim3(256), 0, stream(), A.cols, f.first.p, f.last.p, f.off.p,
                     f.val.p, c);
  f.tiles.release();
  f.tile_off.release();
  f.next_plan.reset();
  return true;
}

bool slab_dot(const DevMat& A, const DevMat& B, double out[2]) {
  if (!sa_operand(A) || !sa_operand(B) || A.cols != B.cols) return false;
  const int n = A.cols;
  const SlabForm &fa = *A.slab, &fb = *B.slab;
  DevBuf<double> part((size_t)2 * n), res(2);
  hipLaunchKernelGGL(k_sa_dot, dim3(cdiv((int64_t)n * WAVE, 256)), dim3(256), 0, stream(), n, fa.first.p, fa.last.p, fa.off.p, fa.val.p,
                     fb.first.p, fb.last.p, fb.off.p, fb.val.p, part.p);
  reduce_sum2_async(part.p, n, res.p);
  unsigned long long h[2] = {0, 0};
  ScalarFetch ft;
  ft.add(res.p, 2, h);
  ft.run();
  std::memcpy(out, h, sizeof(h));
  return true;
}

bool slab_norm(const DevMat& A, double* out) {
  if (!sa_operand(A)) return false;
  const SlabForm& f = *A.slab;
  DevBuf<double> cs((size_t)A.cols);
  hipLaunchKernelGGL(k_sa_colstat<double>, dim3(cdiv((int64_t)A.cols * WAVE, 256)), dim3(256), 0, stream(), A.cols, f.first.p, f.last.p, f.off.p,
                     f.val.p, 0, 0, cs.p, (double*)nullptr);
  *out = max_of(cs, (size_t)A.cols);
  return true;
}

bool slab_gershgorin(const DevMat& A, int32_t col_offset, double* mn, double* mx) {
  if (!sa_operand(A)) return false;
  const SlabForm& f = *A.slab;
  DevBuf<double> lo((size_t)A.cols), hi((size_t)A.cols), res(2);
  hipLaunchKernelGGL(k_sa_colstat<double>, dim3(cdiv((int64_t)A.cols * WAVE, 256)), dim3(256), 0, stream(), A.cols, f.first.p, f.last.p, f.off.p,
                     f.val.p, col_offset, 1, lo.p, hi.p);
  launch_reduce_minmax(lo.p, hi.p, (int64_t)A.cols, res.p);
  double h[2];
  res.download(h, 2);
  *mn = h[0];
  *mx = h[1];
  return true;
}

namespace {
__global__ __launch_bounds__(256) void k_sa_tiles(int n, const int32_t* __restrict__ first, const int32_t* __restrict__ last,
                                                  const int64_t* __restrict__ off, const double* __restrict__ val,
                                                  const int32_t* __restrict__ blk_kmin, const int32_t* __restrict__ blk_kn,
                                                  const int64_t* __restrict__ boff, double* __restrict__ tiles, int nblocks) {
  const int b = xcd_block(nblocks);
  if (b < 0) return;
  const int kmin = blk_kmin[b], kn = blk_kn[b], kn2 = (kn + 1) & ~1;
  const int c = threadIdx.x & 15, j = b * SLAB_J + c;
  const bool colv = j < n;
  const int f = colv ? first[j] : INT_MAX, l = colv ? last[j] : -1;
  const double* __restrict__ p = (colv && l >= f) ? val + (off[j] - f) : val;
  double* __restrict__ dst = tiles + boff[b];
  for (int idx = threadIdx.x; idx < kn2 * SLAB_J; idx += 256) {
    const int r = kmin + (idx >> 4);
    dst[idx] = (r >= f && r <= l) ? p[r] : 0.0;
  }
}
struct EmptyDot {
  DevBuf<int32_t> dmin, dmax;
  DevBuf<int64_t> doff;
  DevBuf<double> dexp;
  int n = 0;
};
const EmptyDot& empty_dot(int n) {
  static EmptyDot* e = new EmptyDot();
  if (e->n < n) {
    e->dmin.alloc((size_t)n); e->dmax.alloc((size_t)n); e->doff.alloc((size_t)n + 1); e->dexp.alloc(8);
    std::vector<int32_t> hmin((size_t)n, INT_MAX), hmax((size_t)n, -1);
    e->dmin.upload(hmin.data(), (size_t)n);
    e->dmax.upload(hmax.data(), (size_t)n);
    sync_stream();
    e->doff.zero();
    e->dexp.zero();
    e->n = n;
  }
  return *e;
}

bool slab_multiply_loop(const DevMat& A, const DevMat& B, DevMat& C, double alpha, double threshold, bool dense_rule) {
// ... 583 lines not shown
```

### ntpoly_amd/csrc/kernels.hpp

```cpp
#pragma once
#include <functional>
#include "common.hpp"

namespace ntp {

struct SpgemmStats {
  int64_t nnz_a = 0, nnz_b = 0, nnz_c = 0;
  int64_t products = 0;
  int64_t tmp_entries = 0;
  int slab = 0;
  int fused = 0;
  int64_t bin_cols[6] = {0, 0, 0, 0, 0, 0};
  int64_t overflow_cols = 0;
  int grouped = 0;
  int strips = 0;
  int64_t gh_failed_cols = 0, gh_groups = 0, gh_tile_rows = 0;
  int gh_level = 0, gh_minhash = 0;
  double gh_union_ratio = 0;
  int block = 0;
  double block_fill = 0;
  int64_t block_tile_products = 0, block_cand = 0;
  int thin = 0;
  float ms_total = 0.f;
  float ms_numeric = 0.f;
};

struct EngineOptions {
  int spgemm_force_bin = -1;
  int increment_force_seq = 0;
  int time_kernels = 0;
  int spgemm_fma = 1;
  int block_path = 1;
  int slab_algebra = 1;
  int plan_ahead = 1;
  int operand_cache = 1;
  int tile_rows = 2;
  int tile_waves = 0;
  int thin_left = 1;
 int complex_sessions = 1;
  int column_fused = 1;
  int complex_tile = 1;
  int block_complex = 1;
  int tile2 = 0;
  int tile_runs_only = 1;
  int load_balance = 1;
  int virtual_grid = 0;
  int fused_update = 1;
  int block_scope = 1;
  int block_scope_complex = 1;
  int block_match = 0;
  int block_unfused = 0;
  int panel_sessions = 1;
  int thin_slab_complex = 1;
  int complex_poly_sessions = 2;
  int complex_panels = 1;
  int complex_density = 1;
  int ghash_mfma = 1;
  int tile_off32 = 1;
  int tile_bbuf = 2;
  int plan_fused = 1;
  int exchange_ahead = 1;
  int band_scope = 1;
  int label_order = 1;
  int label_rowoff = 1;
  int loose_iterates = 1;
  int halo_overlap = 1;
  int spgemm_variant = -1;
};
EngineOptions& options();
SpgemmStats& last_spgemm_stats();
struct SpgemmAccum { int64_t calls = 0, products = 0, nnz_c = 0; double alg_bytes = 0, ms_numeric = 0, ms_total = 0; };
SpgemmAccum& spgemm_accum();
void flush_spgemm_timers();

struct LooseProduct {
  bool valid = false;
  int32_t rows = 0, cols = 0;
  int64_t slots = 0;
  DevBuf<int64_t> start;
  DevBuf<int32_t> count;
  DevBuf<int32_t> inner;
  DevBuf<double> val;
  DevBuf<int64_t> prod_scan;
  int64_t prod_index = -1;
};

struct ColRange { int32_t a, b; };
struct SlabFusion {
  int mode = 0;
  double am = 0, bm = 0, threshold = 0;
  const DevMat* D = nullptr;
  int32_t col_offset = 0;
  int32_t panel_c0 = -1;
  bool done = false;
  DevMat result;
  double dot = 0, trace = 0;
  int64_t product_nnz = 0;
  int64_t refused = 0;
};
void spgemm(const DevMat& A, const DevMat& B, DevMat& C, double alpha, double threshold,
            bool dense_rule, LooseProduct* loose = nullptr, const ColRange* arange = nullptr, SlabFusion* fuse = nullptr);
bool trs2_block_step(DevMat& X, int mode, double threshold, bool dense_rule, const DevMat& D, double out[4]);
struct BlockKeepScope {
  BlockKeepScope();
  ~BlockKeepScope();
  BlockKeepScope(const BlockKeepScope&) = delete;
  BlockKeepScope& operator=(const BlockKeepScope&) = delete;
};
struct SlabReduce {
  void (*allreduce)(double* dev4) = nullptr;
  double reduced[4] = {0, 0, 0, 0};
  bool done = false;
};
struct SlabHalo {
  int32_t ka = 0, kb = 0;
  const int32_t* first = nullptr;
  const int32_t* last = nullptr;
  const unsigned long long* addr = nullptr;
  const int32_t* count = nullptr;
  int row_pad = 1;
  SlabReduce* reduce = nullptr;
  std::function<void(const DevMat& result, const long long* d_nnz, ScalarFetch& fetch)> before_fetch;
  SlabPlan* plan = nullptr;
  int thin = 0;
  int64_t nnz_a = 0;
  std::function<void(ScalarFetch& fetch)> on_fetch;
};
bool slab_plan_fits_tile(int max_kn, int max_w);
struct SlabPlan;
bool slab_multiply_takes_panel(const DevMat& A, const DevMat& B, int left_row_pad, int32_t ka, int32_t kb, const SlabPlan* plan);
void slab_plan_panel_async(const DevMat& X, const int64_t* d_ext_all, int pitch, int32_t dim, int P, SlabPlan& plan,
                           DevBuf<int32_t>& gfirst, DevBuf<int32_t>& glast, unsigned long long* stats24);
bool slab_step(DevMat& X, SlabFusion& fuse, double threshold, bool dense_rule, const SlabHalo* halo = nullptr);
void slab_request_async(const DevMat& X, int64_t* d_out4, const long long* d_nnz = nullptr);
void slab_extents_async(const DevMat& X, int64_t* d_ext, int64_t* d_pre);
void slab_pack_runs_async(const DevMat& X, const int64_t* d_pre, int32_t ja, int32_t jb, double* dst);
void slab_halo_layout_async(const int64_t* d_ext_all, const int64_t* d_pre_all, int pitch, int32_t dim, int P, int me,
                            int32_t ka, int32_t kb, const int32_t* d_ra, const int64_t* d_zoff, const double* d_recv,
                            const DevMat& X, int32_t* d_first, int32_t* d_last, unsigned long long* d_addr,
                            const int64_t* d_cnt_all = nullptr, int32_t* d_count = nullptr,
                            const int32_t* h_ra = nullptr, const int64_t* h_zoff = nullptr);
void slab_export_async(const DevMat& X, int64_t* d_out4, const long long* d_nnz, int64_t* d_ext, int64_t* d_pre, int64_t* d_cnt64);
void slab_counts_async(const DevMat& X, int64_t* d_cnt64);
bool slab_enter(DevMat& M);
bool slab_multiply(const DevMat& A, const DevMat& B, DevMat& C, double alpha, double threshold, bool dense_rule, const SlabHalo* left = nullptr);
inline bool block_arithmetic_ok() { return options().spgemm_fma == 1 || (options().spgemm_fma == 0 && options().block_unfused != 0); }
bool slab_panels_ok();
void slab_allow_panels(bool on);
bool sa_operand_c(const DevMat& M);
bool slab_enter_c(DevMat& M, bool* not_run_like = nullptr);
bool slab_multiply_c(const DevMat& A, const DevMat& B, DevMat& C, double alpha, double threshold, bool dense_rule, const SlabHalo* left = nullptr);
bool slab_multiply_c_takes_panel(const DevMat& A, const DevMat& B, int left_row_pad, int32_t ka, int32_t kb, const SlabPlan* plan);
bool slab_add_diagonal_c(DevMat& B, double alpha, int32_t col_offset);
bool slab_norm_axpby_c(const DevMat& A, const DevMat& B, double alpha, double beta, double* out);
bool slab_recurrence_step_c(const DevMat& P, const DevMat& Tkm2, DevMat& Tk, DevMat& R, double a, double c);
bool slab_dot_trace_c(const DevMat& A, const DevMat* B, int32_t col_offset, double dot[2], double* trace);
bool slab_axpby(const DevMat& A, DevMat& B, double alpha, double beta, double threshold);
bool slab_axpby_to(const DevMat& A, const DevMat& B, DevMat& Out, double alpha, double beta, double threshold);
bool slab_clone(const DevMat& A, DevMat& Out);
bool slab_scale(DevMat& A, double c);
bool slab_dot(const DevMat& A, const DevMat& B, double out[2]);
bool slab_norm(const DevMat& A, double* out);
bool slab_axpby_c(const DevMat& A, DevMat& B, double alpha, double beta, double threshold);
bool slab_axpby_to_c(const DevMat& A, const DevMat& B, DevMat& Out, double alpha, double beta, double threshold);
bool slab_clone_c(const DevMat& A, DevMat& Out);
bool slab_scale_c(DevMat& A, double c);
bool slab_norm_c(const DevMat& A, double* out);
bool slab_gershgorin(const DevMat& A, int32_t col_offset, double* mn, double* mx);
bool slab_add_diagonal(DevMat& B, double alpha, int32_t col_offset);
bool slab_trs4_traces(const DevMat& X, const DevMat& X2, int32_t col_offset, double* trace_fx, double* trace_gx);
bool slab_trs4_operand(const DevMat& X, const DevMat& X2, double sigma, int32_t col_offset, DevMat& Out);
bool slab_norm_axpby(const DevMat& A, const DevMat& B, double alpha, double beta, double* out);
bool slab_trace(const DevMat& A, int32_t col_offset, double* out);
int64_t slab_span_sum(const DevMat& M);
long long slab_product_count(const DevMat& A, const DevMat& B);
bool slab_from_csc(DevMat& Xs, DevBuf<int32_t>& lab);
bool relabel_enter(DevMat& X, const DevMat& D);
const DevMat* relabelled_operand(const DevMat& D);
void relabel_giveup(const DevMat& D);
void drop_thin_transposes();
void drop_operand_caches();
void set_scope_labels(const int32_t* lab);
const int32_t* scope_labels();
void drop_pending_exchange();
bool find_band_order(const DevMat& A, DevBuf<int32_t>& newpos, int64_t* bandwidth);
int64_t column_span_sum(const DevMat& A);
unsigned long long pattern_fingerprint_of(const DevMat& A);
long long* fusion_counts();
long long* complex_fusion_counts();
long long* tile2_counts();
long long& band_searches();

void increment(const DevMat& A, DevMat& B, double alpha, double threshold);
void increment_blocked(const DevMat& A, DevMat& B, double alpha, double threshold, int32_t row_block);
void axpby(const DevMat& A, DevMat& B, double alpha, double beta, double threshold, const DevMat* D, double* dot_out,
           double* trace_out = nullptr, int32_t trace_col_offset = 0);
void axpby(const LooseProduct& A, DevMat& B, double alpha, double beta, double threshold, const DevMat* D, double* dot_out,
           double* trace_out, int32_t trace_col_offset, int64_t* a_nnz_out, bool keep_loose = false);
DevMat packed_copy(const DevMat& M);
void pack(DevMat& M);
bool square_keep_loose(DevMat& X, double threshold, bool dense_rule, const DevMat& D, double out[2], double* trace_out,
                       int32_t col_offset);
void pairwise(const DevMat& A, const DevMat& B, DevMat& C, bool conj_a);
void dot(const DevMat& A, const DevMat& B, double out[2]);
void dot_trace(const DevMat& A, const DevMat& B, double out[2], double* trace_out, int32_t col_offset);
void grand_sum(const DevMat& A, double out[2]);
double trace(const DevMat& A, int32_t col_offset);
void column_abs_sums(const DevMat& A, DevBuf<double>& out);
double max_of(const DevBuf<double>& v, size_t n);
void gershgorin(const DevMat& A, int32_t col_offset, double* mn, double* mx);
void scale(DevMat& A, double c);
void conjugate(DevMat& A);
void scale_columns(DevMat& A, const double* d_factor);
DevMat to_complex(const DevMat& A);
DevMat to_real(const DevMat& A);
DevMat identity(int32_t n, int32_t col_offset, int32_t cols, bool cplx);
int64_t identity_check(const DevMat& A, int32_t col_offset);
DevMat transpose(const DevMat& A);
DevMat remap_general(const DevMat& A, const int32_t* d_row_map, const int32_t* d_col_map, int32_t new_rows,
                     int32_t col_lo, int32_t col_hi, bool drop_exact_zeros);
DevMat transpose_slice(const DevMat& A, int32_t col_lo, int32_t col_hi);
DevMat column_slice(const DevMat& A, int32_t c0, int32_t c1);
DevMat mask_columns(const DevMat& A, int32_t col_offset, int32_t block, int32_t slices, int32_t slice);
DevMat concat_columns(const std::vector<const DevMat*>& parts);

DevMat from_triplets(const HostTriplets& t, int32_t rows, int32_t cols, int32_t col_offset);
void to_triplets(const DevMat& A, int32_t col_offset, HostTriplets& out);

void copy_shift_i64(const int64_t* d_src, int64_t* d_dst, int64_t count, int64_t shift);

void rebase_i64(const int64_t* d_src, int64_t* d_dst, int64_t count, int64_t add);
void fill_i64(int64_t* d_dst, int64_t count, int64_t v);
void row_range(const DevMat& A, int32_t* lo, int32_t* hi);
void halo_request_async(const DevMat& B, int64_t nnz_a, int64_t* d_out4);
void halo_interior_async(const DevMat& B, int32_t c0, int32_t c1, int64_t* d_out5);
void halo_counts_async(const int64_t* d_req, const int64_t* d_outer_all, int pitch, int32_t dim, int P, int me, int64_t* d_cnt,
                       int64_t* d_bound);
void halo_bounds_async(const DevMat& A, int32_t c0, const int32_t* d_sa, const int32_t* d_sb, int P, int64_t* d_bound,
                       int64_t* d_cnt_row);

bool spgemm_thin_left(const DevMat& A, const DevMat& B, DevMat& C, double alpha, double threshold, int dense_rule_bits, int64_t* products,
                      hipEvent_t ev_begin, hipEvent_t ev_end);
struct ThinSlabArgs {
  const int32_t *blk_lo = nullptr, *blk_w = nullptr;
  const int64_t* blk_toff = nullptr;
  const int32_t *bfirst = nullptr, *blast = nullptr;
  const int64_t* boff = nullptr;
  const double* bval = nullptr;
  const int32_t *afirst = nullptr, *alast = nullptr;
  const int64_t* aoff = nullptr;
  const double* aval = nullptr;
  const int64_t* at_outer = nullptr;
  const int32_t* at_inner = nullptr;
  const double* at_val = nullptr;
  double* out_val = nullptr;
  int32_t *count = nullptr, *ofirst = nullptr, *olast = nullptr;
  int64_t* ooff = nullptr;
  double alpha = 1.0, threshold = 0.0;
  int dense_rule = 0, ncols = 0, nrows = 0;
  int* flag = nullptr;
  const unsigned long long* aaddr = nullptr;
  int nblocks = 0;
};
void launch_thin_slab(const ThinSlabArgs& a, bool left, bool cplx = false);
struct ThinRows {
  DevBuf<int64_t> outer;
  DevBuf<int32_t> inner;
  DevBuf<double> val;
};
void thin_rows_from_runs(bool cplx, const int32_t* first, const int32_t* last, const unsigned long long* addr, const int64_t* off,
                         const double* base, int32_t ka, int32_t kb, int32_t nrows, int64_t cap, ThinRows& out);
inline int slab_thin_rule(int64_t nnz_a, int64_t nnz_b, int64_t dim) {
  return (nnz_a <= 8 * dim && nnz_b >= nnz_a) ? 1 : (nnz_b <= 8 * dim) ? 2 : 0;
// ... 18 lines not shown
```

### ntpoly_amd/csrc/spgemm_tile.hip

```cpp
#include "spgemm_tile.hpp"
#include <string>

#include <hip/hip_runtime.h>

#include <cstdio>
#include <cstdlib>
#include <vector>

#include "device_util.hpp"
#include "kernels.hpp"

namespace ntp {
namespace {

typedef double v4d __attribute__((ext_vector_type(4)));
typedef double v2d __attribute__((ext_vector_type(2)));
template <int R> struct RowVec;
template <> struct RowVec<1> { typedef double type; };
template <> struct RowVec<2> { typedef v2d type; };
template <> struct RowVec<4> { typedef v4d type; };
template <int R> __device__ inline double rv_get(const typename RowVec<R>::type& x, int m) { return x[m]; }
template <> __device__ inline double rv_get<1>(const double& x, int) { return x; }
template <int R> __device__ inline void rv_set(typename RowVec<R>::type& x, int m, double v) { x[m] = v; }
template <> __device__ inline void rv_set<1>(double& x, int, double v) { x = v; }
template <int R> __device__ inline typename RowVec<R>::type rv_load(unsigned long long addr) {
  return *reinterpret_cast<const typename RowVec<R>::type __attribute__((address_space(1)))*>(addr);
}
template <int R> __device__ inline typename RowVec<R>::type rv_load(const double* p) { return rv_load<R>(reinterpret_cast<unsigned long long>(p)); }
template <int R> __device__ inline void rv_store(double* p, const typename RowVec<R>::type& v) {
  *reinterpret_cast<typename RowVec<R>::type __attribute__((address_space(1)))*>(reinterpret_cast<unsigned long long>(p)) = v;
}

typedef unsigned v4u __attribute__((ext_vector_type(4)));
typedef unsigned v2u __attribute__((ext_vector_type(2)));
constexpr unsigned TILE_OOB = 0xffffff00u;
template <int R> __device__ inline typename RowVec<R>::type rv_buffer_load(__amdgpu_buffer_rsrc_t rsrc, unsigned off);
template <> __device__ inline double rv_buffer_load<1>(__amdgpu_buffer_rsrc_t rsrc, unsigned off) {
  return __builtin_bit_cast(double, __builtin_amdgcn_raw_buffer_load_b64(rsrc, off, 0, 0));
}
template <> __device__ inline v2d rv_buffer_load<2>(__amdgpu_buffer_rsrc_t rsrc, unsigned off) {
  return __builtin_bit_cast(v2d, __builtin_amdgcn_raw_buffer_load_b128(rsrc, off, 0, 0));
}
template <> __device__ inline v4d rv_buffer_load<4>(__amdgpu_buffer_rsrc_t rsrc, unsigned off) {
  const v2d lo = __builtin_bit_cast(v2d, __builtin_amdgcn_raw_buffer_load_b128(rsrc, off, 0, 0));
  const v2d hi = __builtin_bit_cast(v2d, __builtin_amdgcn_raw_buffer_load_b128(rsrc, off + 16u, 0, 0));
  return v4d{lo[0], lo[1], hi[0], hi[1]};
}

struct alignas(16) TileRec {
  unsigned long long rz;
  int32_t first;
  uint32_t span;
};
#ifndef NTP_TILE_PF
#define NTP_TILE_PF 6
#endif
constexpr int TILE_PF = NTP_TILE_PF;
constexpr int TILE_RPAD = 4;
__host__ __device__ constexpr int tile_bp(bool) { return 17; }
__host__ __device__ constexpr int tile_bpad(bool) { return 2; }
struct alignas(16) TileDefer {
  int32_t r, jj, prow, pad;
  double o, d;
};
constexpr int TILE_DEFER = 48;


struct TileArgs {
  const SlabRun* runs;
  const double* bblk;
  const int64_t* blk_boff;
  const int32_t *blk_kmin, *blk_kn, *blk_lo, *blk_w;
  const int64_t* blk_toff;
  double* out_val;
  int32_t* count;
  int32_t *ofirst, *olast;
  int64_t* ooff;
  int64_t* otoff;
  double alpha, threshold;
  int dense_rule, ncols, nblocks;
  int nrows;
  int k4max, tmax;
  SlabFuseArgs fzv;
  const int32_t *brun_first, *brun_last;
  const int64_t* brun_off;
  const double* brun_val;
  int bpair;
  uint32_t bbytes;
  const double* zero;
  const void* abase;
  uint32_t abytes;
  const void* dbase;
  uint32_t dbytes;
  int ablate;
#ifdef NTP_TILE_STAMPS
  long long* stamps;
  long long* blkdur;
#endif
};

__host__ __device__ inline size_t tile_lds_bytes(int k4max, int tmax, int lab_rows = 0) {
  return (size_t)lab_rows * 4 + (size_t)(k4max + tile_bpad(lab_rows > 0)) * tile_bp(lab_rows > 0) * 8 + (size_t)(k4max + TILE_RPAD) * sizeof(TileRec) + (size_t)tmax * 4 + (size_t)(k4max / 4 + 1) * 8 + 16 + TILE_DEFER * sizeof(TileDefer) + 16 * 5 * 4 +
         2 * 8 * 8 + (size_t)tmax * 16 + 8 + (size_t)(k4max + 8) * 4 + 64;
}

#ifdef NTP_TILE_STAMPS
#define STAMP(i) do { if (lane == 0 && b % 97 == 0 && b / 97 < 64 && (i) < 64) a.stamps[((b / 97) * 8 + wave) * 64 + (i)] = __builtin_amdgcn_s_memtime(); } while (0)
#else
#define STAMP(i) do { } while (0)
#endif

template <int EPI, int TILE_NW, int R, bool LAB, bool OFF32>
#ifdef NTP_TILE_WPE3
__global__ __launch_bounds__(TILE_NW* WAVE) __attribute__((amdgpu_waves_per_eu((((EPI == 0 || !LAB) && R <= 2) && TILE_NW != 4) ? 4 : 3, 8))) void k_spgemm_tile(const TileArgs a) {
#else
__global__ __launch_bounds__(TILE_NW* WAVE) __attribute__((amdgpu_waves_per_eu(R <= 2 ? 4 : 3, 8))) void k_spgemm_tile(const TileArgs a) {
#endif
  extern __shared__ __attribute__((aligned(16))) char smem[];
  constexpr bool LABK = LAB && EPI != 0;
  constexpr int BP = tile_bp(LABK), BPAD = tile_bpad(LABK);
  const int b = xcd_block(a.nblocks);
  if (b < 0) return;
  const int tid = threadIdx.x, wave = uni_i32(tid / WAVE), lane = lane_id();
  const int lo = a.blk_lo[b], w = a.blk_w[b], kmin = a.blk_kmin[b], kn = a.blk_kn[b];
  const int64_t tbase = a.blk_toff[b];
  const bool brun = a.brun_val != nullptr;
  int bf0 = INT_MAX, bl0 = -1, bf1 = INT_MAX, bl1 = -1;
  const double *bp0 = nullptr, *bp1 = nullptr;
  unsigned bo0 = 0u, bo1 = 0u;
  auto thread_extents = [&]() {
    const int c0 = b * SLAB_J + 2 * (tid & 7);
    if (c0 < a.ncols) {
      bf0 = a.brun_first[c0]; bl0 = a.brun_last[c0];
      const int64_t o = a.brun_off[c0];
      bp0 = a.brun_val + (o - bf0);
      bo0 = ((unsigned)o - (unsigned)bf0) * 8u;
    }
    if (c0 + 1 < a.ncols) {
      bf1 = a.brun_first[c0 + 1]; bl1 = a.brun_last[c0 + 1];
      const int64_t o = a.brun_off[c0 + 1];
      bp1 = a.brun_val + (o - bf1);
      bo1 = ((unsigned)o - (unsigned)bf1) * 8u;
    }
  };
  constexpr bool PAIR_OK = (TILE_NW == 4 || TILE_NW == 8) && BPAD == 2;
  constexpr int CPW = PAIR_OK ? SLAB_J / TILE_NW : 1;
  [[maybe_unused]] int cbf[CPW], cbl[CPW];
  [[maybe_unused]] unsigned cbo[CPW];
  const bool bpair = PAIR_OK && brun && a.bbytes != 0u && a.bpair != 0;
  if (bpair) {
#pragma unroll
    for (int m = 0; m < CPW; ++m) {
      const int c = b * SLAB_J + CPW * wave + m;
      cbf[m] = INT_MAX; cbl[m] = -1; cbo[m] = 0u;
      if (c < a.ncols) {
        cbf[m] = a.brun_first[c]; cbl[m] = a.brun_last[c];
        cbo[m] = ((unsigned)a.brun_off[c] - (unsigned)cbf[m]) * 8u;
      }
    }
  } else if (brun) thread_extents();
  [[maybe_unused]] int e_raw = 0, e_xpl = -1;
  [[maybe_unused]] int64_t e_raw8 = 0;
  if constexpr (EPI != 0) {
    const int jc0 = min(b * SLAB_J + (tid & 15), a.ncols - 1);
    const int sel = (tid >> 4) & 3;
    if constexpr (EPI == 2) {
      const int32_t* p4 = sel == 0 ? a.fzv.dmin : sel == 1 ? a.fzv.dmax : sel == 2 ? a.fzv.xmin : a.fzv.xmax;
      const int64_t* p8 = (sel & 1) ? a.fzv.xoff : a.fzv.doff;
      e_raw = p4[jc0];
      e_raw8 = p8[jc0];
      if constexpr (LAB) e_xpl = a.fzv.xplast[jc0];
    } else {
      const int32_t* p4 = (sel & 1) ? a.fzv.dmax : a.fzv.dmin;
      e_raw = p4[jc0];
      e_raw8 = a.fzv.doff[jc0];
    }
  }
  if (b == 0 && tid == 0) {
    a.ooff[a.ncols] = a.blk_toff[a.nblocks];
    if (EPI != 0 && a.otoff) a.otoff[a.nblocks] = a.blk_toff[a.nblocks];
  }
  if (kn == 0) {
    const int j = b * SLAB_J + tid;
    if (tid < SLAB_J && j < a.ncols) {
      a.ofirst[j] = INT_MAX;
      a.olast[j] = -1;
      a.count[j] = 0;
      a.ooff[j] = tbase + (int64_t)tid * w;
      if constexpr (EPI != 0) {
        if (a.fzv.oplast) a.fzv.oplast[j] = -1;
        if (EPI == 2 && a.fzv.xmax[j] >= a.fzv.xmin[j]) atomicOr(a.fzv.flag, 1);
      }
    }
    if (EPI != 0 && tid == 0) a.otoff[b] = tbase;
    return;
  }
  STAMP(0);
#ifdef NTP_TILE_STAMPS
  if (tid == 0 && a.blkdur) a.blkdur[4 * b] = __builtin_amdgcn_s_memtime();
#endif
  double* Bs = reinterpret_cast<double*>(smem) + (BPAD / 2) * BP;
  TileRec* recs = reinterpret_cast<TileRec*>(reinterpret_cast<double*>(smem) + (size_t)(a.k4max + BPAD) * BP);
  int* grmin = reinterpret_cast<int*>(recs + a.k4max + TILE_RPAD);
  int* grmax = grmin + (a.k4max / 4 + 1);
  unsigned* colmask = reinterpret_cast<unsigned*>(grmax + (a.k4max / 4 + 1));
  TileDefer* dlist = reinterpret_cast<TileDefer*>(colmask + ((a.tmax + 2 * (a.k4max / 4 + 1) + 3) & ~3) - 2 * (a.k4max / 4 + 1));
  int* col_cnt = reinterpret_cast<int*>(dlist + TILE_DEFER);
  int* col_first = col_cnt + 16;
  int* col_last = col_first + 16;
  int* col_pmax = col_last + 16;
  int* col_plast = col_pmax + 16;
  double* red = reinterpret_cast<double*>(col_plast + 16);
  double* tred = red + 2 * 8;
  int* misc = reinterpret_cast<int*>(tred + 2 * a.tmax);
  [[maybe_unused]] int* cntl = misc + 6 + 1;
  [[maybe_unused]] int* labs = misc + 6 + (a.k4max + 8);

  const int KG = (kn + 3) >> 2, K4 = KG * 4;
  constexpr int TROWS = 16 * R;
  typedef typename RowVec<R>::type VR;
  const int T = (w + TROWS - 1) / TROWS;
  if (kn > 0 && w > 0 && tbase >= 0) STAMP(56);
  constexpr int NT = TILE_NW * WAVE, BCH = 3072 / NT;
  const double2* __restrict__ bsrc = reinterpret_cast<const double2*>(a.bblk + (a.blk_boff ? a.blk_boff[b] : 0));
  double2 btmp[BCH];
  auto brun_load = [&](int i) {
    const int r = kmin + (i >> 3);
    double2 v;
#ifdef NTP_ABL_NOBLOAD
    v.x = (i < kn * 8 && r >= bf0 && r <= bl0) ? 1.0 : 0.0;
    v.y = (i < kn * 8 && r >= bf1 && r <= bl1) ? 1.0 : 0.0;
    return v;
#endif
    v.x = (i < kn * 8 && r >= bf0 && r <= bl0) ? bp0[r] : 0.0;
    v.y = (i < kn * 8 && r >= bf1 && r <= bl1) ? bp1[r] : 0.0;
    return v;
  };
  [[maybe_unused]] int bcnt[BCH];
  [[maybe_unused]] const int32_t* __restrict__ prod_count = nullptr;
  [[maybe_unused]] bool want_prod = false;
  if constexpr (EPI != 0) {
    want_prod = a.fzv.prod != nullptr;
    prod_count = a.fzv.in_count;
  }
#ifndef NTP_TILE_NO_RECFIRST
  constexpr int RCH = (384 + 4 + NT - 1) / NT;
  uint4 rh0[RCH], rh1[RCH];
  {
    const uint4* __restrict__ rp_h = reinterpret_cast<const uint4*>(a.runs + kmin);
#pragma unroll
    for (int u = 0; u < RCH; ++u) {
      const int ic = min(tid + u * NT, kn - 1);
      rh0[u] = rp_h[2 * ic];
      rh1[u] = rp_h[2 * ic + 1];
    }
  }
  STAMP(50);
#ifdef NTP_TILE_STAMPS
  if (brun && bf0 + bl0 + bf1 + bl1 == 0x7ffffff1) STAMP(59);
  STAMP(52);
#endif
#endif
  const int bpath = (brun && a.bbytes != 0u) ? ((bpair && K4 + 2 <= 384) ? 2 : 1) : 0;
  if (bpath != 2 && bpair) thread_extents();
  constexpr int CCH = (384 + NT - 1) / NT;
  [[maybe_unused]] int ctmp[CCH];
  if constexpr (EPI != 0) {
    if (bpath == 2 && want_prod) {
      const int32_t* __restrict__ pc = prod_count;
      const int rmax = kmin + kn - 1;
#pragma unroll
// ... 530 lines not shown
    if constexpr (EPI == 2) {
      if (pm_l >= 0) atomicMax(&col_pmax[jj], pm_l);
    }
    if ((cm >> jj) & 1u) {
#pragma unroll
      for (int v = 0; v < 4; ++v) rv_store<R>(orun + (r0 + R * (4 * v + q)), res[v]);
    }
    if constexpr (EPI != 0) {
      if (cm && otile) {
#pragma unroll
        for (int v = 0; v < 4; ++v) {
#pragma unroll
          for (int m = 0; m < R; ++m) otile[(int64_t)(r0 + R * (4 * v + q) + m) * SLAB_J] = rv_get<R>(res[v], m);
        }
      }
    }
    if (lane == 0) colmask[t] = cm;
#ifndef NTP_TILE_STATIC
    if constexpr (EPI != 0) {
      const double td = wave_sum_f64(dsum), tt = wave_sum_f64(tsum);
      if (lane == 0) {
        tred[2 * t] = td;
        tred[2 * t + 1] = tt;
      }
    }
#endif
    STAMP(sidx); ++sidx;
  }
  STAMP(2);
#ifdef NTP_TILE_STATIC
  if constexpr (EPI != 0) {
    dsum = wave_sum_f64(dsum);
    tsum = wave_sum_f64(tsum);
    if (lane == 0) {
      red[2 * wave] = dsum;
      red[2 * wave + 1] = tsum;
    }
  }
#endif
  if (lane == 0 && pn) atomicAdd(&misc[1], pn);
  __syncthreads();
  STAMP(3);
  if constexpr (EPI == 2) {
    const int nd = misc[0];
    if (nd != 0) {
    if (nd > TILE_DEFER) {
      if (tid == 0) atomicOr(a.fzv.flag, 1);
    } else {
      for (int i = tid; i < nd; i += TILE_NW * WAVE) {
        const int4 e = *reinterpret_cast<const int4*>(&dlist[i]);
        const bool kept = e.z > col_pmax[e.y];
        if (kept) {
          atomicAdd(&col_cnt[e.y], 1);
          atomicMin(&col_first[e.y], e.x);
          atomicMax(&col_last[e.y], e.x);
          if constexpr (LAB) atomicMax(&col_plast[e.y], e.z);
        }
        dlist[i].pad = kept ? 1 : 0;
      }
    }
    __syncthreads();
    if (nd <= TILE_DEFER && tid < nd) {
      const TileDefer e = dlist[tid];
      if (e.pad) {
        int rank = 0;
        for (int m2 = 0; m2 < nd; ++m2) {
          const TileDefer f = dlist[m2];
          rank += (f.pad && (f.r < e.r || (f.r == e.r && f.jj < e.jj))) ? 1 : 0;
        }
        Bs[rank] = __dmul_rn(e.o, e.d);
        Bs[TILE_DEFER + rank] = (e.r == b * SLAB_J + e.jj + a.fzv.col_offset) ? e.o : 0.0;
      }
    }
    __syncthreads();
    }
  }
  if (tid < SLAB_J) {
    const int jt = b * SLAB_J + tid;
    const int cf = col_first[tid], cl = col_last[tid];
    if (jt < a.ncols) {
      a.count[jt] = col_cnt[tid];
      a.ofirst[jt] = cf;
      a.olast[jt] = cl;
      a.ooff[jt] = tbase + (int64_t)tid * w + (cl >= cf ? cf - lo : 0);
      if constexpr (EPI != 0) {
        if constexpr (LAB) a.fzv.oplast[jt] = col_plast[tid];
      }
    }
  }
  int tk0 = INT_MAX, tk1 = -1;
#pragma unroll
  for (int c = 0; c < SLAB_J; ++c) {
    tk0 = min(tk0, col_first[c]);
    tk1 = max(tk1, col_last[c]);
  }
  if constexpr (EPI != 0) {
    if (tid == 0) {
      a.otoff[b] = tbase + (tk1 >= tk0 ? (int64_t)(tk0 - lo) * SLAB_J : 0);
      a.fzv.pnnz[b] = misc[1];
      if (a.fzv.prod) a.fzv.prod[b] = *reinterpret_cast<long long*>(misc + 2);
    }
    if (tid == 64) {
      double x = 0.0, y = 0.0;
#ifdef NTP_TILE_STATIC
      for (int qq = 0; qq < TILE_NW; ++qq) {
        x = __dadd_rn(x, red[2 * qq]);
        y = __dadd_rn(y, red[2 * qq + 1]);
      }
#else
      for (int t2 = 0; t2 < T; ++t2) {
        x = __dadd_rn(x, tred[2 * t2]);
        y = __dadd_rn(y, tred[2 * t2 + 1]);
      }
#endif
      if constexpr (EPI == 2) {
        const int nd = min(misc[0], TILE_DEFER);
        int nk = 0;
        for (int m2 = 0; m2 < nd; ++m2) nk += dlist[m2].pad;
        for (int m2 = 0; m2 < nk; ++m2) {
          x = __dadd_rn(x, Bs[m2]);
          y = __dadd_rn(y, Bs[TILE_DEFER + m2]);
        }
      }
      a.fzv.part[2 * b] = x;
      a.fzv.part[2 * b + 1] = y;
    }
  }
  for (int p = tid; p < T * SLAB_J; p += TILE_NW * WAVE) {
    const int t = p >> 4, c = p & 15;
    const unsigned cmk = colmask[t];
    const int cf = col_first[c], cl = col_last[c];
    const int r0 = lo + TROWS * t;
    if (cl >= cf && r0 + TROWS - 1 >= cf && r0 <= cl && !((cmk >> c) & 1u)) {
      double* dst = a.out_val + (tbase + (int64_t)c * w - lo);
      for (int r = r0; r < min(r0 + TROWS, rend); ++r) dst[r] = 0.0;
    }
    if constexpr (EPI != 0) {
      if (a.fzv.tiles && tk1 >= tk0 && r0 + TROWS - 1 >= tk0 && r0 <= tk1 && cmk == 0u) {
        double* dst = a.fzv.tiles + (tbase - (int64_t)lo * SLAB_J + c);
        for (int r = r0; r < min(r0 + TROWS, rend); ++r) dst[(int64_t)r * SLAB_J] = 0.0;
      }
    }
  }
  if constexpr (EPI == 2) {
    const int nd = min(misc[0], TILE_DEFER);
    if (nd > 0) {
      __syncthreads();
      for (int i = tid; i < nd; i += TILE_NW * WAVE) {
        const TileDefer e = dlist[i];
        if (!e.pad) continue;
        a.out_val[tbase + (int64_t)e.jj * w + (e.r - lo)] = e.o;
        if (a.fzv.tiles) a.fzv.tiles[tbase + (int64_t)(e.r - lo) * SLAB_J + e.jj] = e.o;
      }
    }
  }
  STAMP(55);
#ifdef NTP_TILE_STAMPS
  if (tid == 0 && a.blkdur) {
    a.blkdur[4 * b + 1] = __builtin_amdgcn_s_memtime();
    a.blkdur[4 * b + 2] = EPI == 2 ? misc[0] : 0;
    a.blkdur[4 * b + 3] = kn;
  }
#endif
}

}

#ifndef NTP_WITH_TILE2
bool launch_spgemm_tile2(const TileLaunch&, int*) { return false; }
#endif

int tile_rows() {
  const int r = options().tile_rows;
  return r == 4 ? 4 : r == 1 ? 1 : 2;
}

bool spgemm_tile_fits(int max_kn, int max_w) {
  const int k4 = std::max(8, (max_kn + 3) & ~3), tm = (max_w + 15) >> 4;
  return max_kn > 0 && max_w > 0 && std::max(tile_lds_bytes(k4, tm, 16 * tm + 64), tile_lds_bytes(k4, tm, 0)) <= 150 * 1024;
}

void launch_spgemm_tile(const TileLaunch& L) {
  TileArgs a;
  a.runs = static_cast<const SlabRun*>(L.runs);
  a.bblk = L.bblk; a.blk_boff = L.blk_boff; a.blk_kmin = L.blk_kmin; a.blk_kn = L.blk_kn; a.blk_lo = L.blk_lo; a.blk_w = L.blk_w;
  a.blk_toff = L.blk_toff; a.out_val = L.out_val; a.count = L.count; a.ofirst = L.ofirst; a.olast = L.olast; a.ooff = L.ooff;
  a.otoff = L.otoff; a.alpha = L.alpha; a.threshold = L.threshold; a.dense_rule = L.dense_rule; a.ncols = L.ncols;
  a.nblocks = L.nblocks;
  a.nrows = L.nrows > 0 ? L.nrows : L.ncols;
  a.k4max = std::max(8, (L.max_kn + 3) & ~3);
  const int trows = 16 * (L.rows == 4 ? 4 : L.rows == 2 ? 2 : 1);
  a.tmax = (L.max_w + trows - 1) / trows;
  if (L.fz) a.fzv = *static_cast<const SlabFuseArgs*>(L.fz);
  a.brun_first = L.brun_first; a.brun_last = L.brun_last; a.brun_off = L.brun_off; a.brun_val = L.brun_val;
  a.bbytes = (options().tile_bbuf != 0 && L.brun_val && L.bbytes > 0 && L.bbytes < 0xffffe000ull) ? (uint32_t)L.bbytes : 0u;
  a.bpair = (a.bbytes != 0u && options().tile_bbuf >= 2 && L.brun_pad >= 2 && L.brun_pad % 2 == 0) ? 1 : 0;
  static DevBuf<double>* zeros = nullptr;
  if (!zeros) {
    zeros = new DevBuf<double>(8);
    zeros->zero();
  }
  a.zero = zeros->p;
  bool off32 = options().tile_off32 != 0 && L.abase != nullptr && L.abytes > 0 && L.abytes < 0xfffff000ull;
  if (off32 && L.epi != 0) {
    const SlabFuseArgs& fzh = *static_cast<const SlabFuseArgs*>(L.fz);
    const char *a0 = static_cast<const char*>(L.abase), *x0 = reinterpret_cast<const char*>(fzh.xexp);
    off32 = L.dbase != nullptr && L.dbytes > 0 && L.dbytes < 0xfffff000ull && (L.epi != 2 || (x0 >= a0 && x0 < a0 + L.abytes));
  }
  a.abase = off32 ? L.abase : nullptr;
  a.abytes = off32 ? (uint32_t)L.abytes : 0u;
  a.dbase = off32 ? L.dbase : nullptr;
  a.dbytes = off32 ? (uint32_t)L.dbytes : 0u;
  a.ablate = options().spgemm_variant == 601 ? 1 : options().spgemm_variant == 602 ? 2 : 0;
#ifdef NTP_TILE_STAMPS
  static DevBuf<long long>* stamps = nullptr;
  if (!stamps) stamps = new DevBuf<long long>(64 * 8 * 64);
  stamps->zero();
  a.stamps = stamps->p;
  static DevBuf<long long>* blkdur = nullptr;
  if (!blkdur || blkdur->n < (size_t)4 * L.nblocks) { delete blkdur; blkdur = new DevBuf<long long>((size_t)4 * L.nblocks); }
  blkdur->zero();
  a.blkdur = blkdur->p;
#endif
  const size_t lds = tile_lds_bytes(a.k4max, a.tmax, (L.labelled && L.epi != 0) ? a.tmax * trows : 0);
#ifdef NTP_TILE_WIDE3
  const bool wide = 3 * ((lds + 511) & ~(size_t)511) > 160 * 1024;
#else
  const bool wide = 4 * ((lds + 511) & ~(size_t)511) > 160 * 1024;
#endif
  const int tw = options().tile_waves;
  const int nw = (tw == 4 || tw == 5 || tw == 6 || tw == 8) ? tw : (wide ? 8 : 4);
  auto go = [&](auto epi_tag, auto nw_tag, auto r_tag, auto lab_tag, auto off_tag) {
    constexpr int E = decltype(epi_tag)::value, NW = decltype(nw_tag)::value, RR = decltype(r_tag)::value;
    constexpr bool LB = decltype(lab_tag)::value, OF = decltype(off_tag)::value;
    static size_t raised = 0;
    if (lds > 64 * 1024 && lds > raised) {
      HIP_CHECK(hipFuncSetAttribute(reinterpret_cast<const void*>(&k_spgemm_tile<E, NW, RR, LB, OF>), hipFuncAttributeMaxDynamicSharedMemorySize,
                                    150 * 1024));
      raised = 150 * 1024;
    }
    hipLaunchKernelGGL((k_spgemm_tile<E, NW, RR, LB, OF>), dim3(xcd_grid(L.nblocks)), dim3(NW * WAVE), lds, stream(), a);
  };
  auto by_off = [&](auto epi_tag, auto nw_tag, auto r_tag, auto lab_tag) {
    constexpr int NW = decltype(nw_tag)::value, RR = decltype(r_tag)::value;
    if constexpr ((NW == 4 || NW == 8) && RR <= 2) {
      if (off32) return go(epi_tag, nw_tag, r_tag, lab_tag, std::true_type{});
    }
    go(epi_tag, nw_tag, r_tag, lab_tag, std::false_type{});
  };
  auto by_nw = [&](auto epi_tag, auto r_tag, auto lab_tag) {
    if (nw == 4) by_off(epi_tag, std::integral_constant<int, 4>{}, r_tag, lab_tag);
    else if (nw == 5) by_off(epi_tag, std::integral_constant<int, 5>{}, r_tag, lab_tag);
    else if (nw == 6) by_off(epi_tag, std::integral_constant<int, 6>{}, r_tag, lab_tag);
    else by_off(epi_tag, std::integral_constant<int, 8>{}, r_tag, lab_tag);
  };
  auto by_r = [&](auto epi_tag) {
    constexpr int E = decltype(epi_tag)::value;
    using F = std::false_type; using T = std::true_type;
    using R1 = std::integral_constant<int, 1>; using R2 = std::integral_constant<int, 2>; using R4 = std::integral_constant<int, 4>;
    if constexpr (E != 0) {
      if (L.labelled) {
        if (L.rows >= 2) by_nw(epi_tag, R2{}, T{});
        else by_nw(epi_tag, R1{}, T{});
        return;
      }
    }
    if (L.rows == 4) by_nw(epi_tag, R4{}, F{});
    else if (L.rows == 2) by_nw(epi_tag, R2{}, F{});
    else by_nw(epi_tag, R1{}, F{});
  };
// ... 18 lines not shown
```

### ntpoly_amd/csrc/spgemm_tile.hpp

```cpp
#pragma once
#include "slab_types.hpp"

namespace ntp {

struct TileLaunch {
  const void* runs = nullptr;
  const double* bblk = nullptr;
  const int64_t* blk_boff = nullptr;
  const int32_t *blk_kmin = nullptr, *blk_kn = nullptr, *blk_lo = nullptr, *blk_w = nullptr;
  const int64_t* blk_toff = nullptr;
  double* out_val = nullptr;
  int32_t* count = nullptr;
  int32_t *ofirst = nullptr, *olast = nullptr;
  int64_t* ooff = nullptr;
  int64_t* otoff = nullptr;
  double alpha = 1.0, threshold = 0.0;
  int dense_rule = 0, ncols = 0, nblocks = 0;
  int max_kn = 0, max_w = 0;
  int epi = 0;
  int rows = 1;
  const void* fz = nullptr;
  const int32_t *brun_first = nullptr, *brun_last = nullptr;
  const int64_t* brun_off = nullptr;
  const double* brun_val = nullptr;
  size_t bbytes = 0;
  int brun_pad = 1;
  const void* abase = nullptr;
  size_t abytes = 0;
  const void* dbase = nullptr;
  size_t dbytes = 0;
  int nrows = 0;
  bool labelled = false;
};
bool spgemm_tile_fits(int max_kn, int max_w);
int tile_rows();
inline int tile_expand_align() { return 16 * tile_rows(); }
void launch_spgemm_tile(const TileLaunch& a);
bool launch_spgemm_tile2(const TileLaunch& a, int* fail);
bool spgemm_tile_c_fits(int max_kn, int max_w);
void launch_spgemm_tile_c(const TileLaunch& a);

}
```

### ntpoly_amd/csrc/wrp.cpp

```cpp
#include <algorithm>
#include <cmath>
#include <cstring>

#include "engine.hpp"
#include "spgemm_block.hpp"
#include "io.hpp"

using namespace ntp;

namespace {
constexpr int SIZE_wrp = 12;

template <typename T>
T* get(const int* ih) {
  T* p;
  std::memcpy(&p, ih, sizeof(p));
  if (!p) NTP_FATAL("null handle passed to the C ABI");
  return p;
}
PSMatrix* get_unpacked(const int* ih) {
  PSMatrix* p;
  std::memcpy(&p, ih, sizeof(p));
  if (!p) NTP_FATAL("null handle passed to the C ABI");
  return p;
// ... 27 lines not shown
  if (!global_grid_constructed()) NTP_FATAL("the global process grid has not been constructed");
  return &global_grid();
}
std::string fstring(const char* s, const int* n) { return std::string(s, (size_t)*n); }

void local_diagonal_scale(DevMat& m, const HostTriplets& t) {
  if (m.cols == 0) return;
  const size_t w = m.wval();
  std::vector<double> f((size_t)m.cols * w, 0.0);
  for (int32_t j = 0; j < m.cols; ++j) f[(size_t)j * w] = 1.0;
  for (size_t i = 0; i < t.size(); ++i) {
    const int32_t col = t.col[i] - 1;
    if (col < 0 || col >= m.cols) continue;
    const double re = t.cplx ? t.val[2 * i] : t.val[i], im = t.cplx ? t.val[2 * i + 1] : 0.0;
    double& fr = f[(size_t)col * w];
    if (m.cplx) {
      double& fi = f[(size_t)col * w + 1];
      const double nr = fr * re - fi * im, ni = fr * im + fi * re;
      fr = nr;
      fi = ni;
    } else {
      fr *= re;
    }
  }
  DevBuf<double> d(f.size());
  d.upload(f.data(), f.size());
  scale_columns(m, d.p);
  sync_stream();
}
void local_print(const DevMat& m, const char* path) {
  HostTriplets t;
  to_triplets(m, 0, t);
  FILE* f = path ? std::fopen(path, "w") : stdout;
  if (!f) NTP_FATAL(std::string("cannot open ") + path + " for writing");
  std::fprintf(f, "%%%%MatrixMarket matrix coordinate %s general\n%%\n", m.cplx ? "complex" : "real");
  std::fprintf(f, "%d %d %lld\n", m.rows, m.cols, (long long)m.nnz);
  for (size_t i = 0; i < t.size(); ++i) {
    if (m.cplx) std::fprintf(f, "%d %d %.17g %.17g\n", t.row[i], t.col[i], t.val[2 * i], t.val[2 * i + 1]);
    else std::fprintf(f, "%d %d %.17g\n", t.row[i], t.col[i], t.val[i]);
  }
  if (path) std::fclose(f);
  else std::fflush(f);
}
std::unique_ptr<SlabSession> g_test_session;
}

extern "C" {

void ntpoly_amd_get_unique_id(char* out128) { comm_get_unique_id(out128); }
void ntpoly_amd_init_comm(const char* id128, const int* rank, const int* nranks) { comm_init(id128, *rank, *nranks); }
void ntpoly_amd_finalize_comm() { comm_finalize(); }
int ntpoly_amd_comm_rank() { return base_world().rank; }
int ntpoly_amd_comm_size() { return base_world().nranks; }
void ntpoly_amd_barrier() { comm_barrier(); }
void ntpoly_amd_allreduce_max(double* values, const int* n) { comm_allreduce_max(values, *n); }
void ntpoly_amd_synchronize() {
  ensure_init();
  sync_stream();
  HIP_CHECK(hipDeviceSynchronize());
}
int ntpoly_amd_device_count() {
  int n = 0;
  if (hipGetDeviceCount(&n) != hipSuccess) return 0;
  return n;
}
void ntpoly_amd_panel_range(const int* dim, const int* nranks, const int* rank, int* c0, int* c1) {
  panel_range(*dim, *nranks, *rank, c0, c1);
}
void ntpoly_amd_halo_segment(const int* dim, const int* nranks, const int* s, const int* kmin, const int* kmax, int* a,
                             int* b) {
  halo_segment(*dim, *nranks, *s, *kmin, *kmax, a, b);
}
void ntpoly_amd_panel_exchange_layout(const int* dim, const int* nranks, const int* me, const long long* req, const long long* cnt,
                                      int* sa, int* sb, long long* soff, int* ra, int* rb, long long* zoff) {
  panel_exchange_layout(*dim, *nranks, *me, reinterpret_cast<const int64_t*>(req), reinterpret_cast<const int64_t*>(cnt), sa, sb,
                        reinterpret_cast<int64_t*>(soff), ra, rb, reinterpret_cast<int64_t*>(zoff));
}
void ntpoly_amd_set_option(const char* name, const int* value) {
  const std::string n(name);
  if (n == "spgemm_force_bin") options().spgemm_force_bin = *value;
  else if (n == "increment_force_seq") options().increment_force_seq = *value;
  else if (n == "spgemm_fma") options().spgemm_fma = *value;
  else if (n == "plan_ahead") options().plan_ahead = *value;
  else if (n == "slab_algebra") options().slab_algebra = *value;
  else if (n == "operand_cache") options().operand_cache = *value;
  else if (n == "tile_rows") options().tile_rows = *value;
  else if (n == "tile_waves") options().tile_waves = *value;
  else if (n == "time_kernels") options().time_kernels = *value;
  else if (n == "spgemm_variant") options().spgemm_variant = *value;
  else if (n == "halo_overlap") options().halo_overlap = *value;
  else if (n == "load_balance") options().load_balance = *value;
  else if (n == "virtual_grid") options().virtual_grid = *value;
  else if (n == "loose_iterates") options().loose_iterates = *value;
  else if (n == "fused_update") options().fused_update = *value;
  else if (n == "label_order") options().label_order = *value;
  else if (n == "band_scope") options().band_scope = *value;
  else if (n == "exchange_ahead") options().exchange_ahead = *value;
  else if (n == "plan_fused") options().plan_fused = *value;
  else if (n == "tile_off32") options().tile_off32 = *value;
  else if (n == "tile_bbuf") options().tile_bbuf = *value;
  else if (n == "ghash_mfma") options().ghash_mfma = *value;
  else if (n == "block_unfused") options().block_unfused = *value;
  else if (n == "block_match") options().block_match = *value;
  else if (n == "block_scope") options().block_scope = *value;
  else if (n == "block_scope_complex") options().block_scope_complex = *value;
  else if (n == "panel_sessions") options().panel_sessions = *value;
  else if (n == "complex_panels") options().complex_panels = *value;
  else if (n == "complex_density") options().complex_density = *value;
  else if (n == "label_rowoff") options().label_rowoff = *value;
  else if (n == "block_path") options().block_path = *value;
  else if (n == "tile_runs_only") options().tile_runs_only = *value;
  else if (n == "tile2") options().tile2 = *value;
  else if (n == "complex_tile") options().complex_tile = *value;
  else if (n == "block_complex") options().block_complex = *value;
  else if (n == "thin_left") options().thin_left = *value;
  else if (n == "thin_slab_complex") options().thin_slab_complex = *value;
  else if (n == "complex_poly_sessions") options().complex_poly_sessions = *value;
  else if (n == "column_fused") options().column_fused = *value;
  else if (n == "complex_sessions") options().complex_sessions = *value;
  else NTP_FATAL("unknown option " + n);
}
int ntpoly_amd_get_option(const char* name) {
  const std::string n(name);
  if (n == "spgemm_fma") return options().spgemm_fma;
  if (n == "slab_algebra") return options().slab_algebra;
  if (n == "plan_ahead") return options().plan_ahead;
  if (n == "tile_rows") return options().tile_rows;
  if (n == "tile2") return options().tile2;
  if (n == "block_path") return options().block_path;
  if (n == "label_order") return options().label_order;
  if (n == "band_scope") return options().band_scope;
  if (n == "exchange_ahead") return options().exchange_ahead;
  if (n == "plan_fused") return options().plan_fused;
  if (n == "tile_off32") return options().tile_off32;
  if (n == "tile_bbuf") return options().tile_bbuf;
  if (n == "ghash_mfma") return options().ghash_mfma;
  if (n == "block_unfused") return options().block_unfused;
  if (n == "block_match") return options().block_match;
  if (n == "block_scope") return options().block_scope;
  if (n == "block_scope_complex") return options().block_scope_complex;
  if (n == "panel_sessions") return options().panel_sessions;
  if (n == "complex_panels") return options().complex_panels;
  if (n == "complex_density") return options().complex_density;
  if (n == "fused_update") return options().fused_update;
  if (n == "loose_iterates") return options().loose_iterates;
  if (n == "complex_tile") return options().complex_tile;
  if (n == "block_complex") return options().block_complex;
  if (n == "thin_left") return options().thin_left;
  if (n == "thin_slab_complex") return options().thin_slab_complex;
  if (n == "complex_poly_sessions") return options().complex_poly_sessions;
  if (n == "column_fused") return options().column_fused;
  if (n == "complex_sessions") return options().complex_sessions;
  NTP_FATAL("unknown option " + n);
}
void ntpoly_amd_last_spgemm_stats(long long* out, float* ms_numeric, float* ms_total) {
  flush_spgemm_timers();
  const SpgemmStats& s = last_spgemm_stats();
  out[0] = s.nnz_a; out[1] = s.nnz_b; out[2] = s.nnz_c; out[3] = s.products; out[4] = s.tmp_entries;
  for (int i = 0; i < 6; ++i) out[5 + i] = s.bin_cols[i];
  out[11] = s.overflow_cols;
  out[12] = s.slab;
  *ms_numeric = s.ms_numeric;
  *ms_total = s.ms_total;
}
void ntpoly_amd_last_grouped_stats(long long* out, double* ratio) {
  const SpgemmStats& s = last_spgemm_stats();
  out[0] = s.grouped; out[1] = s.gh_failed_cols; out[2] = s.gh_groups; out[3] = s.gh_level; out[4] = s.gh_minhash;
  out[5] = s.gh_tile_rows;
  *ratio = s.gh_union_ratio;
}
int ntpoly_amd_last_spgemm_thin() { return last_spgemm_stats().thin; }
void ntpoly_amd_thin_slab_counts(long long* out) {
  for (int q = 0; q < 6; ++q) out[q] = thin_slab_counts()[q];
}
void ntpoly_amd_session_begin(const int* complex_ok) {
  if (g_test_session) NTP_FATAL("ntpoly_amd_session_begin: a session is already open");
  g_test_session.reset(new SlabSession(true, false, *complex_ok != 0));
}
void ntpoly_amd_session_end() { g_test_session.reset(); }
int ntpoly_amd_recurrence_step(const int* ih_P, const int* ih_Tkm2, int* ih_Tk, int* ih_R, const double* a, const double* c) {
  return ps_recurrence_step(*get_unpacked(ih_P), *get_unpacked(ih_Tkm2), *get_unpacked(ih_Tk), *get_unpacked(ih_R), *a, *c) ? 1 : 0;
}
void ntpoly_amd_recurrence_step_count(long long* out) { *out = recurrence_step_count(); }
void ntpoly_amd_last_block_stats(long long* out, double* fill) {
  const SpgemmStats& s = last_spgemm_stats();
  out[0] = s.block; out[1] = s.block_tile_products; out[2] = s.block_cand;
  *fill = s.block_fill;
}
int ntpoly_amd_block_order(const int* ih, int* position) {
  PSMatrix& m = *get<PSMatrix>(ih);
  std::vector<int32_t> pos;
  if (!block_order_for(m.loc, pos)) return 0;
  std::memcpy(position, pos.data(), sizeof(int32_t) * pos.size());
  return 1;
}
void ntpoly_amd_drop_block_caches() { drop_block_caches(); }
int ntpoly_amd_block_order_of_pattern(const int* ih, int* position, int* ns) {
  PSMatrix& m = *get<PSMatrix>(ih);
  DevMat full = ps_gather_full(m);
  std::vector<int32_t> pos;
  int32_t s = 0;
  if (!block_order_of_pattern(full, pos, &s)) return 0;
  std::memcpy(position, pos.data(), sizeof(int32_t) * pos.size());
  *ns = s;
  return 1;
}
void ntpoly_amd_exchange_stats(long long* out) {
  out[0] = exchange_stats().exchanges;
  out[1] = exchange_stats().host_syncs;
  out[2] = host_sync_count();
}
int ntpoly_amd_band_order(const int* ih, int* newpos, long long* bandwidth) {
  PSMatrix& m = *get<PSMatrix>(ih);
  DevBuf<int32_t> pos;
  int64_t bw = 0;
  if (!find_band_order(m.loc, pos, &bw)) return 0;
  HIP_CHECK(hipMemcpyAsync(newpos, pos.p, sizeof(int32_t) * (size_t)m.loc.cols, hipMemcpyDeviceToHost, stream()));
  sync_stream();
  *bandwidth = bw;
  return 1;
}
void ntpoly_amd_fusion_counts(long long* out) {
  for (int q = 0; q < 3; ++q) out[q] = fusion_counts()[q];
}
void ntpoly_amd_complex_fusion_counts(long long* out) {
  for (int q = 0; q < 3; ++q) out[q] = complex_fusion_counts()[q];
}
void ntpoly_amd_tile2_counts(long long* out) {
  for (int q = 0; q < 2; ++q) out[q] = tile2_counts()[q];
}
void ntpoly_amd_gather_matrix_to_process(const int* ih_this, int* ih_local, const int* within_slice_id) {
  const PSMatrix& m = *get<PSMatrix>(ih_this);
  DevMat full = ps_gather_full(m);
  const ProcessGrid& g = m.grid ? *m.grid : global_grid();
  const int slice_size = g.num_rows * g.num_cols;
  const int in_slice = g.global_rank - slice_size * g.my_slice;
  if (*within_slice_id >= 0 && *within_slice_id != in_slice) return;
  auto* L = new LocalMat();
  L->m = std::move(full);
  put(ih_local, L);
}
void ntpoly_amd_comm_split_matrix(const int* ih_this, int* ih_split, int* my_color, bool* split_slice) {
  const PSMatrix& m = *get<PSMatrix>(ih_this);
  if (!m.grid) NTP_FATAL("CommSplitMatrix of a matrix that was never constructed");
  auto* out = new PSMatrix();
  ps_comm_split(m, *out, my_color, split_slice);
  put(ih_split, out);
}
void ntpoly_amd_split_process_grid(const int* ih_old_grid, int* ih_new_grid, int* my_color, bool* split_slice) {
  put(ih_new_grid, split_process_grid(*get<ProcessGrid>(ih_old_grid), my_color, split_slice));
}
void ntpoly_amd_grid_comm_info(const int* ih_grid, int* out) {
  const ProcessGrid* g = get<ProcessGrid>(ih_grid);
  out[0] = g->global_rank;
  out[1] = g->total;
  out[2] = g->comm != nullptr ? 1 : 0;
}
void ntpoly_amd_band_scope_counts(long long* out) {
  for (int q = 0; q < 2; ++q) out[q] = band_scope_counts()[q];
}
void ntpoly_amd_block_scope_counts(long long* out) {
  out[0] = band_scope_counts()[2];
  out[1] = block_scope_products();
}
void ntpoly_amd_column_fused_counts(long long* out) {
  out[0] = column_fused_counts()[0];
  out[1] = column_fused_counts()[1];
}
void ntpoly_amd_increment_identity(const int* ih_identity, int* ih_matB, const double* alpha) {
  ps_increment_identity(*get<PSMatrix>(ih_identity), *get<PSMatrix>(ih_matB), *alpha);
}
int ntpoly_amd_norm_axpby(const int* ih_matA, const int* ih_matB, const double* alpha, const double* beta, double* norm) {
  return ps_norm_axpby(*get<PSMatrix>(ih_matA), *get<PSMatrix>(ih_matB), *alpha, *beta, norm) ? 1 : 0;
}
void ntpoly_amd_block_algebra_counts(long long* out) {
  out[0] = block_algebra_counts()[0];
  out[1] = block_algebra_counts()[1];
}
void ntpoly_amd_slab_algebra_counts(long long* out) {
  for (int q = 0; q < 4; ++q) out[q] = slab_algebra_counts()[q];
}
void ntpoly_amd_panel_product_counts(long long* out) {
  out[0] = panel_product_counts()[0];
  out[1] = panel_product_counts()[1];
  out[2] = panel_product_counts()[2];
}
void ntpoly_amd_band_searches(long long* out) { *out = band_searches(); }
void ntpoly_amd_reset_spgemm_accum() {
  flush_spgemm_timers();
  spgemm_accum() = SpgemmAccum();
}
void ntpoly_amd_get_spgemm_accum(long long* out, double* dout) {
  flush_spgemm_timers();
  const SpgemmAccum& a = spgemm_accum();
  out[0] = a.calls; out[1] = a.products; out[2] = a.nnz_c;
  dout[0] = a.alg_bytes; dout[1] = a.ms_numeric; dout[2] = a.ms_total;
}
int ntpoly_amd_trace_iterations() { return last_trace().iterations; }
void ntpoly_amd_trace_get(double* value, double* energy, double* sigma, long long* nnz) {
  const SolverTrace& t = last_trace();
  for (int i = 0; i < t.iterations; ++i) {
    value[i] = t.value[(size_t)i];
    energy[i] = t.energy[(size_t)i];
    sigma[i] = t.sigma[(size_t)i];
    nnz[i] = t.nnz[(size_t)i];
  }
}
void ntpoly_amd_trace_times(double* setup_ms, double* loop_ms) {
  *setup_ms = last_trace().setup_ms;
  *loop_ms = last_trace().loop_ms;
}
void ntpoly_amd_memory(long long* in_use, long long* cached) {
// ... 815 lines not shown
```

### ntpoly_amd/host.py

```python
import contextlib
import ctypes as C

import numpy as np

from . import capi
from .capi import b, d, handle, i, lib, ll, s


def ConstructGlobalProcessGrid(process_rows=None, process_columns=None, process_slices=None, world_comm=0):
    if process_rows is None and process_slices is None:
        lib.ConstructGlobalProcessGrid_default_wrp(i(world_comm))
    elif process_rows is None:
        lib.ConstructGlobalProcessGrid_onlyslice_wrp(i(world_comm), i(process_slices))
    else:
        lib.ConstructGlobalProcessGrid_wrp(i(world_comm), i(process_rows), i(process_columns), i(process_slices))


def WriteGridInfo():
    lib.WriteGlobalProcessGridInfo_wrp()


def DestructGlobalProcessGrid():
    lib.DestructGlobalProcessGrid_wrp()

# ... 758 lines not shown

    SquareRoot = staticmethod(lambda a, o, p: DenseSolvers._f("DenseSquareRoot_wrp", a, o, p))
    InverseSquareRoot = staticmethod(lambda a, o, p: DenseSolvers._f("DenseInverseSquareRoot_wrp", a, o, p))
    Exponential = staticmethod(lambda a, o, p: DenseSolvers._f("ComputeDenseExponential_wrp", a, o, p))
    Logarithm = staticmethod(lambda a, o, p: DenseSolvers._f("ComputeDenseLogarithm_wrp", a, o, p))
    Sine = staticmethod(lambda a, o, p: DenseSolvers._f("DenseSine_wrp", a, o, p))
    Cosine = staticmethod(lambda a, o, p: DenseSolvers._f("DenseCosine_wrp", a, o, p))
    Invert = staticmethod(lambda a, o, p: DenseSolvers._f("DenseInvert_wrp", a, o, p))
    SignFunction = staticmethod(lambda a, o, p: DenseSolvers._f("DenseSignFunction_wrp", a, o, p))


class LoadBalancer:
    @staticmethod
    def PermuteMatrix(mat_in, mat_out, permutation, memorypool=None):
        pool = memorypool if memorypool is not None else PMatrixMemoryPool(mat_in)
        lib.PermuteMatrix_wrp(mat_in.ih, mat_out.ih, permutation.ih, pool.ih)

    @staticmethod
    def UndoPermuteMatrix(mat_in, mat_out, permutation, memorypool=None):
        pool = memorypool if memorypool is not None else PMatrixMemoryPool(mat_in)
        lib.UndoPermuteMatrix_wrp(mat_in.ih, mat_out.ih, permutation.ih, pool.ih)


class EigenBounds:
    @staticmethod
    def PowerBounds(matrix, solver_parameters):
        v = C.c_double()
        lib.PowerBounds_wrp(matrix.ih, C.byref(v), solver_parameters.ih)
        return v.value

    @staticmethod
    def GershgorinBounds(matrix):
        mn, mx = C.c_double(), C.c_double()
        lib.GershgorinBounds_wrp(matrix.ih, C.byref(mn), C.byref(mx))
        return mn.value, mx.value


def ActivateLogger(start_document=False, file_name=None):
    if file_name:
        raw, n = s(file_name)
        lib.ActivateLoggerFile_wrp(b(start_document), raw, n)
    else:
        lib.ActivateLogger_wrp(b(start_document))


def DeactivateLogger():
    lib.DeactivateLogger_wrp()


def last_spgemm_stats():
    out = (C.c_longlong * 13)()
    a, t = C.c_float(), C.c_float()
    lib.ntpoly_amd_last_spgemm_stats(out, C.byref(a), C.byref(t))
    return dict(nnz_a=out[0], nnz_b=out[1], nnz_c=out[2], products=out[3], tmp_entries=out[4],
                bins=[out[5 + k] for k in range(6)], overflow=out[11], slab=out[12], ms_numeric=a.value, ms_total=t.value)


def band_order(M):
    pos = np.zeros(M.GetActualDimension(), dtype=np.int32)
    bw = C.c_longlong()
    lib.ntpoly_amd_band_order.restype = C.c_int
    ok = lib.ntpoly_amd_band_order(M.ih, pos.ctypes.data_as(C.c_void_p), C.byref(bw))
    return (pos, int(bw.value)) if ok else None


def fusion_counts():
    out = (C.c_longlong * 3)()
    lib.ntpoly_amd_fusion_counts(out)
    return dict(square=out[0], update=out[1], repeated=out[2])


def complex_fusion_counts():
    out = (C.c_longlong * 3)()
    lib.ntpoly_amd_complex_fusion_counts(out)
    return dict(square=out[0], update=out[1], repeated=out[2])


def tile2_counts():
    out = (C.c_longlong * 2)()
    lib.ntpoly_amd_tile2_counts(out)
    return dict(done=out[0], repeated=out[1])


def band_scope_counts():
    out = (C.c_longlong * 2)()
    lib.ntpoly_amd_band_scope_counts(out)
    return dict(solves=out[0], searched=out[1])


def block_scope_counts():
    out = (C.c_longlong * 2)()
    lib.ntpoly_amd_block_scope_counts(out)
    return dict(solves=out[0], products=out[1])


def band_searches():
    out = C.c_longlong()
    lib.ntpoly_amd_band_searches(C.byref(out))
    return int(out.value)


def slab_algebra_counts():
    out = (C.c_longlong * 4)()
    lib.ntpoly_amd_slab_algebra_counts(out)
    return dict(products=out[0], merges=out[1], others=out[2], refusals=out[3])


def panel_product_counts():
    out = (C.c_longlong * 3)()
    lib.ntpoly_amd_panel_product_counts(out)
    return dict(slab=out[0], declined=out[1], host_syncs=out[2])


def thin_slab_counts():
    out = (C.c_longlong * 6)()
    lib.ntpoly_amd_thin_slab_counts(out)
    return dict(real_left=out[0], real_right=out[1], complex_left=out[2], complex_right=out[3], panel_real=out[4], panel_complex=out[5])


@contextlib.contextmanager
def solver_session(complex_ok=True):
    lib.ntpoly_amd_session_begin(C.byref(C.c_int(1 if complex_ok else 0)))
    try:
        yield
    finally:
        lib.ntpoly_amd_session_end()


def recurrence_step(P, Tkm2, Tk, R, a, c):
    lib.ntpoly_amd_recurrence_step.restype = C.c_int
    return bool(lib.ntpoly_amd_recurrence_step(P.ih, Tkm2.ih, Tk.ih, R.ih, d(a), d(c)))


def recurrence_step_count():
    out = C.c_longlong()
    lib.ntpoly_amd_recurrence_step_count(C.byref(out))
    return int(out.value)


def last_grouped_stats():
    out = (C.c_longlong * 6)()
    r = C.c_double()
    lib.ntpoly_amd_last_grouped_stats(out, C.byref(r))
    return dict(used=int(out[0]), failed_cols=int(out[1]), groups=int(out[2]), level=int(out[3]), minhash=int(out[4]),
                tile_rows=int(out[5]), union_ratio=r.value)


def last_block_stats():
    out = (C.c_longlong * 3)()
    r = C.c_double()
    lib.ntpoly_amd_last_block_stats(out, C.byref(r))
    return dict(used=int(out[0]), tile_products=int(out[1]), candidates=int(out[2]), fill=r.value)


def last_spgemm_thin():
    lib.ntpoly_amd_last_spgemm_thin.restype = C.c_int
    return int(lib.ntpoly_amd_last_spgemm_thin())


def block_order(M):
    pos = np.zeros(M.GetActualDimension(), dtype=np.int32)
    lib.ntpoly_amd_block_order.restype = C.c_int
    ok = lib.ntpoly_amd_block_order(M.ih, pos.ctypes.data_as(C.c_void_p))
    return pos if ok else None


# ... 81 lines not shown
```

Measured before the change: 678.8.

## Prepare next SpGEMM step's plan, runs and zero buffers ahead via pinned host slots

Adds a step-ahead mode in the fused slab TRS2 square. The tile kernel now writes the next iteration's SlabRun descriptors directly. The next plan's offsets kernel publishes its sizes into mapped pinned host memory, and the next zero-word buffer is cleared inside the plan kernel. The totals kernel also writes its scalars to mapped host memory, and the host waits on events instead of doing ScalarFetch copies. The aim is to remove per-iteration kernel launches, memsets and blocking device-to-host readbacks. The cost is pooled pinned slots, extra device memory held between steps, and added validity checks via allocation serials.

```diff
diff --git a/include/ntpoly_amd.h b/include/ntpoly_amd.h
--- a/include/ntpoly_amd.h
+++ b/include/ntpoly_amd.h
@@ -82,6 +82,7 @@
 void ntpoly_amd_slab_algebra_counts(long long* out);
 void ntpoly_amd_split_process_grid(const int* ih_old_grid, int* ih_new_grid, int* my_color, bool* split_slice);
 void ntpoly_amd_square_root_order(const int* ih_Input, int* ih_Output, const int* ih_solver_parameters, const int* inverse, const int* order);
+void ntpoly_amd_step_ahead_counts(long long* out);
 void ntpoly_amd_synchronize();
 void ntpoly_amd_thin_slab_counts(long long* out);
 void ntpoly_amd_tile2_counts(long long* out);
diff --git a/ntpoly_amd/csrc/common.cpp b/ntpoly_amd/csrc/common.cpp
--- a/ntpoly_amd/csrc/common.cpp
+++ b/ntpoly_amd/csrc/common.cpp
@@ -5,6 +5,7 @@
 
 #include <cstring>
 #include <mutex>
+#include <vector>
 
 namespace ntp {
 
@@ -69,6 +70,68 @@
   c.calls += 1;
   c.ms += ms;
   c.slow += ms > 10.0 ? 1 : 0;
+}
+
+void sync_event(hipEvent_t e) {
+  host_sync_count() += 1;
+  SyncClock& c = sync_clock();
+  if (!c.on) {
+    HIP_CHECK(hipEventSynchronize(e));
+    return;
+  }
+  const auto t0 = std::chrono::steady_clock::now();
+  HIP_CHECK(hipEventSynchronize(e));
+  const double ms = std::chrono::duration<double, std::milli>(std::chrono::steady_clock::now() - t0).count();
+  c.calls += 1;
+  c.ms += ms;
+  c.slow += ms > 10.0 ? 1 : 0;
+}
+
+namespace {
+struct PendingPool {
+  std::vector<std::pair<unsigned long long*, unsigned long long*>> slots;
+  std::vector<hipEvent_t> events;
+};
+PendingPool& pending_pool() {
+  static PendingPool* p = new PendingPool();
+  return *p;
+}
+}
+hipEvent_t sync_event_get() {
+  PendingPool& P = pending_pool();
+  if (!P.events.empty()) {
+    hipEvent_t e = P.events.back();
+    P.events.pop_back();
+    return e;
+  }
+  hipEvent_t e;
+  HIP_CHECK(hipEventCreateWithFlags(&e, hipEventDisableTiming));
+  return e;
+}
+void sync_event_put(hipEvent_t e) {
+  if (e) pending_pool().events.push_back(e);
+}
+void PlanPending::acquire() {
+  release();
+  ensure_init();
+  PendingPool& P = pending_pool();
+  if (P.slots.empty()) {
+    unsigned long long *h = nullptr, *d = nullptr;
+    HIP_CHECK(hipHostMalloc(reinterpret_cast<void**>(&h), 64 * 64, hipHostMallocMapped));
+    HIP_CHECK(hipHostGetDevicePointer(reinterpret_cast<void**>(&d), h, 0));
+    std::memset(h, 0, 64 * 64);
+    for (int q = 63; q >= 0; --q) P.slots.push_back({h + 8 * q, d + 8 * q});
+  }
+  host = P.slots.back().first;
+  dev = P.slots.back().second;
+  P.slots.pop_back();
+  ready = sync_event_get();
+}
+void PlanPending::release() {
+  if (host) pending_pool().slots.push_back({host, dev});
+  sync_event_put(ready);
+  host = dev = nullptr;
+  ready = nullptr;
 }
 
 namespace {
diff --git a/ntpoly_amd/csrc/common.hpp b/ntpoly_amd/csrc/common.hpp
--- a/ntpoly_amd/csrc/common.hpp
+++ b/ntpoly_amd/csrc/common.hpp
@@ -32,6 +32,7 @@
 void ensure_init();
 inline hipStream_t stream() { return ctx().stream; }
 void sync_stream();
+void sync_event(hipEvent_t e);
 long long& host_sync_count();
 
 struct ScalarFetch {
@@ -98,12 +99,37 @@
 
 constexpr size_t kIndexSlack = 1024;
 
+struct PlanPending {
+  unsigned long long* host = nullptr;
+  unsigned long long* dev = nullptr;
+  hipEvent_t ready = nullptr;
+  PlanPending() = default;
+  PlanPending(const PlanPending&) = delete;
+  PlanPending& operator=(const PlanPending&) = delete;
+  PlanPending(PlanPending&& o) noexcept : host(o.host), dev(o.dev), ready(o.ready) { o.host = o.dev = nullptr; o.ready = nullptr; }
+  PlanPending& operator=(PlanPending&& o) noexcept {
+    if (this != &o) {
+      release();
+      host = o.host; dev = o.dev; ready = o.ready;
+      o.host = o.dev = nullptr; o.ready = nullptr;
+    }
+    return *this;
+  }
+  ~PlanPending() { release(); }
+  void acquire();
+  void release();
+  bool pending() const { return ready != nullptr; }
+};
+hipEvent_t sync_event_get();
+void sync_event_put(hipEvent_t e);
+
 struct SlabPlan {
   DevBuf<int32_t> blk_lo, blk_w, blk_kmin, blk_kn;
   DevBuf<int64_t> blk_toff;
   int64_t total = 0;
   int max_w = 0, max_kn = 0;
   int align = 0;
+  PlanPending sizes;
 };
 struct SlabForm {
   DevBuf<int32_t> first, last, count;
@@ -113,6 +139,16 @@
   int64_t slots = 0;
   bool no_tile2 = false;
   std::unique_ptr<SlabPlan> next_plan;
+  DevBuf<char> next_runs;
+  const void* runs_val = nullptr;
+  unsigned long long runs_serial = 0;
+  DevBuf<int64_t> next_zwords;
+  void drop_ahead() {
+    next_plan.reset();
+    next_runs.release();
+    runs_val = nullptr; runs_serial = 0;
+    next_zwords.release();
+  }
   std::shared_ptr<struct DevMat> origin;
   mutable int64_t span_sum = -1;
   int row_pad = 1;
diff --git a/ntpoly_amd/csrc/kernels.hip b/ntpoly_amd/csrc/kernels.hip
--- a/ntpoly_amd/csrc/kernels.hip
+++ b/ntpoly_amd/csrc/kernels.hip
@@ -639,9 +639,12 @@
                                                    const int32_t* __restrict__ cmax, int32_t* __restrict__ blk_lo,
                                                    int32_t* __restrict__ blk_w, int32_t* __restrict__ blk_kmin,
                                                    int32_t* __restrict__ blk_kn, int64_t* __restrict__ bsz,
-                                                   int64_t* __restrict__ tsz, int nblocks, int align16 = 0) {
+                                                   int64_t* __restrict__ tsz, int nblocks, int align16 = 0,
+                                                   int64_t* __restrict__ zero_words = nullptr, int64_t nzero = 0) {
   const int b = (blockIdx.x * blockDim.x + threadIdx.x) / WAVE;
   const int lane = lane_id();
+  if (zero_words)
+    for (int64_t i = (int64_t)blockIdx.x * blockDim.x + threadIdx.x; i < nzero; i += (int64_t)gridDim.x * blockDim.x) zero_words[i] = 0;
   if (b < nblocks) {
     const int j = b * J + lane;
     const bool has = lane < J && j < ncols && blast[min(j, ncols - 1)] >= 0;
@@ -688,7 +691,8 @@
 __global__ __launch_bounds__(256) void k_slab_offsets(const int32_t* __restrict__ blk_w, const int32_t* __restrict__ blk_kn,
                                                       const int64_t* __restrict__ tsz, const int64_t* __restrict__ bsz,
                                                       int nblocks, int part, int64_t* __restrict__ toff,
-                                                      int64_t* __restrict__ boff, unsigned long long* __restrict__ stats) {
+                                                      int64_t* __restrict__ boff, unsigned long long* __restrict__ stats,
+                                                      unsigned long long* __restrict__ host_sizes = nullptr) {
   __shared__ long long wsum[2][4];
   __shared__ int wmax[2][4];
   const int lane = lane_id(), wave = threadIdx.x / WAVE;
@@ -759,6 +763,17 @@
   if (threadIdx.x == 0 && stats) {
     atomicMax(&stats[16], (unsigned long long)max(max(wmax[0][0], wmax[0][1]), max(wmax[0][2], wmax[0][3])));
     atomicMax(&stats[17], (unsigned long long)max(max(wmax[1][0], wmax[1][1]), max(wmax[1][2], wmax[1][3])));
+    if (host_sizes) {
+      __threadfence();
+      const unsigned long long parts = (unsigned long long)((nblocks + part - 1) / part);
+      if (atomicAdd(&stats[19], 1ull) + 1ull == parts) {
+        __threadfence();
+        host_sizes[0] = atomicAdd(reinterpret_cast<unsigned long long*>(toff + nblocks), 0ull);
+        host_sizes[1] = atomicMax(&stats[16], 0ull);
+        host_sizes[2] = atomicMax(&stats[17], 0ull);
+        __threadfence_system();
+      }
+    }
   }
 }
 
@@ -2473,6 +2488,7 @@
     if (const char* v = std::getenv("NTPOLY_AMD_TILE_ROWS")) e->tile_rows = std::atoi(v);
     if (const char* v = std::getenv("NTPOLY_AMD_TILE_WAVES")) e->tile_waves = std::atoi(v);
     if (const char* v = std::getenv("NTPOLY_AMD_PLAN_AHEAD")) e->plan_ahead = std::atoi(v);
+    if (const char* v = std::getenv("NTPOLY_AMD_STEP_AHEAD")) e->step_ahead = std::atoi(v);
     if (const char* v = std::getenv("NTPOLY_AMD_SLAB_ALGEBRA")) e->slab_algebra = std::atoi(v);
     if (const char* v = std::getenv("NTPOLY_AMD_PANEL_SESSIONS")) e->panel_sessions = std::atoi(v);
     if (const char* v = std::getenv("NTPOLY_AMD_COMPLEX_PANELS")) e->complex_panels = std::atoi(v);
@@ -2524,7 +2540,8 @@
 __global__ __launch_bounds__(256) void k_fused_totals(const int32_t* __restrict__ count, int n, const long long* __restrict__ a,
                                                       const long long* __restrict__ b, const double* __restrict__ part,
                                                       int m, const double* __restrict__ lvl_in, double* __restrict__ out,
-                                                      int stage) {
+                                                      int stage, const unsigned long long* __restrict__ flag_words = nullptr,
+                                                      unsigned long long* __restrict__ host_out = nullptr) {
   __shared__ long long si[3][4];
   __shared__ double sd[2][4];
   const int wave = threadIdx.x / WAVE, lane = lane_id();
@@ -2561,6 +2578,14 @@
     for (int q = 0; q < 3; ++q) oi[q] = si[q][0] + si[q][1] + si[q][2] + si[q][3];
     od[3] = __dadd_rn(__dadd_rn(sd[0][0], sd[0][1]), __dadd_rn(sd[0][2], sd[0][3]));
     od[4] = __dadd_rn(__dadd_rn(sd[1][0], sd[1][1]), __dadd_rn(sd[1][2], sd[1][3]));
+    if (host_out) {
+      for (int q = 0; q < 3; ++q) host_out[q] = (unsigned long long)oi[q];
+      host_out[3] = (unsigned long long)__double_as_longlong(od[3]);
+      host_out[4] = (unsigned long long)__double_as_longlong(od[4]);
+      host_out[5] = flag_words[0];
+      host_out[6] = flag_words[1];
+      __threadfence_system();
+    }
   }
 }
 
@@ -2757,6 +2782,10 @@
   return c;
 }
 long long* tile2_counts() {
+  static long long c[2] = {0, 0};
+  return c;
+}
+long long* step_ahead_counts() {
   static long long c[2] = {0, 0};
   return c;
 }
@@ -3982,7 +4011,8 @@
 namespace {
 template <int J = SLAB_J>
 void launch_slab_plan(SlabPlan& P, int n, const int32_t* first, const int32_t* last, const int32_t* afirst, const int32_t* alast,
-                      int align, unsigned long long* stats, DevBuf<int64_t>* tile_offsets = nullptr) {
+                      int align, unsigned long long* stats, DevBuf<int64_t>* tile_offsets = nullptr,
+                      unsigned long long* host_sizes = nullptr, int64_t* zero_words = nullptr, int64_t nzero = 0) {
   const int snb = cdiv(n, J);
   P.blk_lo.alloc(snb); P.blk_w.alloc(snb); P.blk_kmin.alloc(snb); P.blk_kn.alloc(snb);
   P.blk_toff.alloc((size_t)snb + 1);
@@ -3990,13 +4020,14 @@
   DevBuf<int64_t> bsz(snb), tsz(snb);
   if (tile_offsets) tile_offsets->alloc((size_t)snb + 1);
   hipLaunchKernelGGL((k_slab_plan<J>), dim3(cdiv((int64_t)snb * WAVE, 256)), dim3(256), 0, stream(), n, first, last, afirst,
-                     alast, P.blk_lo.p, P.blk_w.p, P.blk_kmin.p, P.blk_kn.p, bsz.p, tsz.p, snb, align);
+                     alast, P.blk_lo.p, P.blk_w.p, P.blk_kmin.p, P.blk_kn.p, bsz.p, tsz.p, snb, align, zero_words, nzero);
   if (options().plan_fused != 0) {
     const int part = cdiv(cdiv(snb, kOffParts), 256) * 256;
     hipLaunchKernelGGL(k_slab_offsets, dim3(cdiv(snb, part)), dim3(256), 0, stream(), P.blk_w.p, P.blk_kn.p, tsz.p, bsz.p, snb, part,
-                       P.blk_toff.p, tile_offsets ? tile_offsets->p : (int64_t*)nullptr, stats);
+                       P.blk_toff.p, tile_offsets ? tile_offsets->p : (int64_t*)nullptr, stats, host_sizes);
     return;
   }
+  if (host_sizes) NTP_FATAL("launch_slab_plan: sizes to host memory need plan_fused");
   hipLaunchKernelGGL(k_slab_reduce, dim3(64), dim3(256), 0, stream(), P.blk_w.p, P.blk_kn.p, snb, (const int32_t*)nullptr, 0, stats);
   scan_async<int64_t>(tsz.p, P.blk_toff.p, (int64_t)snb);
   if (tile_offsets) scan_async<int64_t>(bsz.p, tile_offsets->p, (int64_t)snb);
@@ -4021,19 +4052,31 @@
   const DotOperand& dop = dot_operand(*fu.D);
   if (!tile && dop.max_tile > SLAB_DTILE) return false;
   const bool timing = options().time_kernels != 0;
+  const bool ahead = tile && !halo && options().plan_ahead != 0 && options().step_ahead != 0 && options().plan_fused != 0;
   EventTimer t_all(timing), t_num(timing);
   t_all.start();
   SpgemmStats st;
   st.nnz_a = st.nnz_b = X.nnz;
   DevBuf<int32_t> count((size_t)n), ofirst((size_t)n), olast((size_t)n);
   DevBuf<int64_t> tmpoff((size_t)n + 1);
-  DevBuf<int64_t> zwords((size_t)4 * snb + 4 + 48);
-  zwords.zero();
+  const size_t zwords_n = (size_t)4 * snb + 4 + 48;
+  DevBuf<int64_t> zwords;
+  bool found_ahead = ahead;
+  const bool take_zwords = ahead && X.slab->next_zwords.p && X.slab->next_zwords.n == zwords_n;
+  int64_t* zw = nullptr;
+  if (take_zwords) {
+    zw = X.slab->next_zwords.p;
+  } else {
+    zwords.alloc(zwords_n);
+    zwords.zero();
+    zw = zwords.p;
+    found_ahead = false;
+  }
   if (!tile) count.zero();
-  int64_t* fz_flag = zwords.p;
-  int64_t* fz_pnnz = zwords.p + 2;
-  double* fz_part = reinterpret_cast<double*>(zwords.p + 3 + 2 * (size_t)snb);
-  unsigned long long* stats = reinterpret_cast<unsigned long long*>(zwords.p + 4 * (size_t)snb + 4);
+  int64_t* fz_flag = zw;
+  int64_t* fz_pnnz = zw + 2;
+  double* fz_part = reinterpret_cast<double*>(zw + 3 + 2 * (size_t)snb);
+  unsigned long long* stats = reinterpret_cast<unsigned long long*>(zw + 4 * (size_t)snb + 4);
   unsigned long long* next_stats = stats + 24;
   const int ka = halo ? halo->ka : 0, nka = halo ? halo->kb - halo->ka : n;
   const int plan_align = tile ? 16 * tile_rows() : 0;
@@ -4041,6 +4084,13 @@
   SlabPlan* plan = &own_plan;
   if (!halo && in.next_plan && in.next_plan->align == plan_align && (int64_t)in.next_plan->blk_lo.n == snb) {
     plan = in.next_plan.get();
+    if (plan->sizes.pending()) {
+      sync_event(plan->sizes.ready);
+      plan->total = (int64_t)plan->sizes.host[0];
+      plan->max_w = (int)plan->sizes.host[1];
+      plan->max_kn = (int)plan->sizes.host[2];
+      plan->sizes.release();
+    }
   } else if (halo && halo->plan && halo->plan->align == plan_align && (int64_t)halo->plan->blk_lo.n == snb) {
     plan = halo->plan;
   } else {
@@ -4054,6 +4104,7 @@
     f.run();
     own_plan.max_w = (int)hs[0];
     own_plan.max_kn = (int)hs[1];
+    found_ahead = false;
   }
   DevBuf<int32_t>&blk_lo = plan->blk_lo, &blk_w = plan->blk_w, &blk_kmin = plan->blk_kmin, &blk_kn = plan->blk_kn;
   DevBuf<int64_t>& blk_toff = plan->blk_toff;
@@ -4072,13 +4123,23 @@
   if (in.labelled() && (int64_t)hst[1] > 2048) return give_up();
   if (!tile)
     hipLaunchKernelGGL((k_slab_tmpoff<SLAB_J>), dim3(cdiv(n + 1, 256)), dim3(256), 0, stream(), n, blk_w.p, blk_toff.p, tmpoff.p);
-  DevBuf<char> runs(((size_t)nka + 4) * sizeof(SlabRun));
-  if (halo)
-    hipLaunchKernelGGL(k_slab_runs_addr, dim3(cdiv(nka + 4, 256)), dim3(256), 0, stream(), halo->first, halo->last, halo->addr,
-                       (unsigned long long)reinterpret_cast<uintptr_t>(in.val.p), reinterpret_cast<SlabRun*>(runs.p), nka, 8);
-  else
-    hipLaunchKernelGGL(k_slab_runs, dim3(cdiv(n + 4, 256)), dim3(256), 0, stream(), in.first.p, in.last.p, in.off.p,
-                       reinterpret_cast<const char*>(in.val.p), 8, reinterpret_cast<SlabRun*>(runs.p), n);
+  DevBuf<char> runs;
+  const SlabRun* runs_p = nullptr;
+  if (ahead && in.next_runs.p && in.next_runs.n == ((size_t)n + 4) * sizeof(SlabRun) && in.runs_val == in.val.p && in.runs_serial != 0 &&
+      in.runs_serial == dev_alloc_serial(in.val.p)) {
+    runs_p = reinterpret_cast<const SlabRun*>(in.next_runs.p);
+  } else {
+    runs.alloc(((size_t)nka + 4) * sizeof(SlabRun));
+    runs_p = reinterpret_cast<const SlabRun*>(runs.p);
+    found_ahead = false;
+    if (halo)
+      hipLaunchKernelGGL(k_slab_runs_addr, dim3(cdiv(nka + 4, 256)), dim3(256), 0, stream(), halo->first, halo->last, halo->addr,
+                         (unsigned long long)reinterpret_cast<uintptr_t>(in.val.p), reinterpret_cast<SlabRun*>(runs.p), nka, 8);
+    else
+      hipLaunchKernelGGL(k_slab_runs, dim3(cdiv(n + 4, 256)), dim3(256), 0, stream(), in.first.p, in.last.p, in.off.p,
+                         reinterpret_cast<const char*>(in.val.p), 8, reinterpret_cast<SlabRun*>(runs.p), n);
+  }
+  if (ahead) step_ahead_counts()[found_ahead ? 0 : 1] += 1;
   const size_t oslots = (size_t)tmp_total + (size_t)tmp_total / 5 + kIndexSlack;
   const bool runs_only = tile && !halo && options().tile_runs_only != 0;
   DevBuf<double> oval(oslots), otiles(runs_only ? 0 : oslots);
@@ -4089,7 +4150,7 @@
   fz.ofirst = ofirst.p; fz.olast = olast.p; fz.tiles = runs_only ? nullptr : otiles.p;
   fz.part = fz_part; fz.pnnz = reinterpret_cast<long long*>(fz_pnnz); fz.flag = reinterpret_cast<int*>(fz_flag);
   fz.col_offset = fu.col_offset;
-  int64_t* blk_prod = zwords.p + 3 + snb;
+  int64_t* blk_prod = zw + 3 + snb;
   const bool labelled = in.labelled() && !halo && !tile;
   if (in.labelled() && halo) return give_up();
   DevBuf<double> tiles_ord;
@@ -4107,7 +4168,7 @@
     int m = 1;
     while (m < (int)hst[1]) m <<= 1;
     hipLaunchKernelGGL(k_slab_order_steps, dim3(xcd_grid(snb)), dim3(256), (size_t)m * 8, stream(), in.lab.p, blk_kmin.p, blk_kn.p,
-                       in.tile_off.p, in.tiles.p, reinterpret_cast<const SlabRun*>(runs.p), n, tiles_ord.p,
+                       in.tile_off.p, in.tiles.p, runs_p, n, tiles_ord.p,
                        reinterpret_cast<SlabRun*>(blkruns.p), steps.p, snb);
     fz.lab = in.lab.p;
     fz.blkruns = reinterpret_cast<const SlabRun*>(blkruns.p);
@@ -4131,11 +4192,12 @@
     fz_args.upload(reinterpret_cast<const char*>(&fz), sizeof(SlabFuseArgs));
   }
   const int dr = dense_rule ? 1 : 0;
+  if (take_zwords) zwords = std::move(X.slab->next_zwords);
   t_num.start();
   auto launch = [&](auto nw_tag, auto mode_tag, auto epi_tag) {
     constexpr int FNW = decltype(nw_tag)::value;
     hipLaunchKernelGGL((k_spgemm_slab<SLAB_J, SLAB_SL, FNW, decltype(mode_tag)::value, decltype(epi_tag)::value>),
-                       dim3(xcd_grid(snb)), dim3(FNW * WAVE), 0, stream(), reinterpret_cast<const SlabRun*>(runs.p) - ka,
+                       dim3(xcd_grid(snb)), dim3(FNW * WAVE), 0, stream(), runs_p - ka,
                        (labelled && !rowoff) ? tiles_ord.p : in.tiles.p, in.tile_off.p, blk_kmin.p, blk_kn.p, blk_lo.p, blk_w.p, blk_toff.p, (int32_t*)nullptr,
                        oval.p, count.p, 1.0, threshold, dr, n, snb, reinterpret_cast<const SlabFuseArgs*>(fz_args.p));
   };
@@ -4144,12 +4206,17 @@
     else launch(nw_tag, mode_tag, std::integral_constant<int, 2>{});
   };
   DevBuf<int64_t> tile_ooff, tile_otoff;
+  DevBuf<char> next_runs;
   bool used_tile2 = false;
   if (tile) {
     tile_ooff.alloc((size_t)n + 1);
     tile_otoff.alloc((size_t)snb + 1);
     TileLaunch tl;
-    tl.runs = reinterpret_cast<const SlabRun*>(runs.p) - ka;
+    if (ahead) {
+      next_runs.alloc(((size_t)n + 4) * sizeof(SlabRun));
+      tl.next_runs = next_runs.p;
+    }
+    tl.runs = runs_p - ka;
     tl.bblk = in.tiles.p; tl.blk_boff = in.tile_off.p;
     if (in.tiles.p == nullptr || in.tile_off.p == nullptr) {
       tl.bblk = nullptr; tl.blk_boff = nullptr;
@@ -4167,6 +4234,7 @@
     }
     if (!halo && options().tile2 != 0 && !in.no_tile2) used_tile2 = launch_spgemm_tile2(tl, reinterpret_cast<int*>(fz_flag) + 2);
     if (!used_tile2) launch_spgemm_tile(tl);
+    else next_runs.release();
   } else if (rowoff) {
     if (max_w > 6 * SLAB_SL * WAVE) by_mode(std::integral_constant<int, 8>{}, std::integral_constant<int, 9>{});
     else if (max_w > SLAB_NW * SLAB_SL * WAVE) by_mode(std::integral_constant<int, 6>{}, std::integral_constant<int, 9>{});
@@ -4179,8 +4247,20 @@
   hipLaunchKernelGGL(k_fused_totals, dim3(FT_BLOCKS), dim3(256), 0, stream(), count.p, n,
                      reinterpret_cast<const long long*>(fz_pnnz), reinterpret_cast<const long long*>(blk_prod), fz_part, snb,
                      (const double*)nullptr, lvl.p, 0);
+  static unsigned long long *totals_host = nullptr, *totals_dev = nullptr;
+  if (ahead && !totals_host) {
+    HIP_CHECK(hipHostMalloc(reinterpret_cast<void**>(&totals_host), 64, hipHostMallocMapped));
+    HIP_CHECK(hipHostGetDevicePointer(reinterpret_cast<void**>(&totals_dev), totals_host, 0));
+  }
   hipLaunchKernelGGL(k_fused_totals, dim3(1), dim3(256), 0, stream(), (const int32_t*)nullptr, 0, (const long long*)nullptr,
-                     (const long long*)nullptr, (const double*)nullptr, 0, lvl.p, tot.p, 1);
+                     (const long long*)nullptr, (const double*)nullptr, 0, lvl.p, tot.p, 1,
+                     reinterpret_cast<const unsigned long long*>(fz_flag), ahead ? totals_dev : (unsigned long long*)nullptr);
+  hipEvent_t ev_totals = nullptr;
+  if (ahead) {
+    t_all.stop();
+    ev_totals = timing ? t_all.b : sync_event_get();
+    if (!timing) HIP_CHECK(hipEventRecord(ev_totals, stream()));
+  }
   unsigned long long raw[5] = {0, 0, 0, 0, 0};
   int64_t flagv[2] = {0, 0};
   DevBuf<double> red4;
@@ -4191,7 +4271,15 @@
   }
   std::unique_ptr<SlabPlan> next;
   unsigned long long next_hs[3] = {0, 0, 0};
-  if (tile && !halo && options().plan_ahead != 0) {
+  DevBuf<int64_t> next_zwords;
+  if (ahead) {
+    next.reset(new SlabPlan());
+    next->sizes.acquire();
+    next_zwords.alloc(zwords_n);
+    launch_slab_plan(*next, n, ofirst.p, olast.p, ofirst.p, olast.p, plan_align, next_stats, nullptr, next->sizes.dev, next_zwords.p,
+                     (int64_t)zwords_n);
+    HIP_CHECK(hipEventRecord(next->sizes.ready, stream()));
+  } else if (tile && !halo && options().plan_ahead != 0) {
     next.reset(new SlabPlan());
     launch_slab_plan(*next, n, ofirst.p, olast.p, ofirst.p, olast.p, plan_align, next_stats);
   }
@@ -4211,7 +4299,12 @@
   R.slab->val = std::move(oval);
   if (runs_only) { R.slab->tile_off.release(); } else R.slab->tiles = std::move(otiles);
   R.slab->slots = tmp_total;
-  {
+  if (ahead) {
+    sync_event(ev_totals);
+    if (!timing) sync_event_put(ev_totals);
+    std::memcpy(raw, totals_host, sizeof(raw));
+    std::memcpy(flagv, totals_host + 5, sizeof(flagv));
+  } else {
     ScalarFetch f;
     f.add(tot.p, 5, raw);
     f.add(fz_flag, 2, flagv);
@@ -4224,8 +4317,8 @@
     f.run();
     if (red4.p) halo->reduce->done = true;
   }
-  t_all.stop();
-  if (next) {
+  if (!ahead) t_all.stop();
+  if (next && !ahead) {
     next->max_w = (int)next_hs[0];
     next->max_kn = (int)next_hs[1];
   }
@@ -4253,6 +4346,14 @@
   const int64_t nnz_in = X.nnz;
   R.nnz = nnz;
   R.slab->next_plan = std::move(next);
+  if (ahead) {
+    R.slab->next_zwords = std::move(next_zwords);
+    if (next_runs.p) {
+      R.slab->next_runs = std::move(next_runs);
+      R.slab->runs_val = R.slab->val.p;
+      R.slab->runs_serial = dev_alloc_serial(R.slab->val.p);
+    }
+  }
   if (!tile) R.slab->tile_off = std::move(plan->blk_toff);
   if (labelled || tile_labelled) {
     R.slab->lab = std::move(X.slab->lab);
@@ -5911,7 +6012,7 @@
                      f.val.p, c);
   f.tiles.release();
   f.tile_off.release();
-  f.next_plan.reset();
+  f.drop_ahead();
   return true;
 }
 
diff --git a/ntpoly_amd/csrc/kernels.hpp b/ntpoly_amd/csrc/kernels.hpp
--- a/ntpoly_amd/csrc/kernels.hpp
+++ b/ntpoly_amd/csrc/kernels.hpp
@@ -33,6 +33,7 @@
   int block_path = 1;
   int slab_algebra = 1;
   int plan_ahead = 1;
+  int step_ahead = 1;
   int operand_cache = 1;
   int tile_rows = 2;
   int tile_waves = 0;
@@ -189,6 +190,7 @@
 long long* fusion_counts();
 long long* complex_fusion_counts();
 long long* tile2_counts();
+long long* step_ahead_counts();
 long long& band_searches();
 
 void increment(const DevMat& A, DevMat& B, double alpha, double threshold);
diff --git a/ntpoly_amd/csrc/spgemm_tile.hip b/ntpoly_amd/csrc/spgemm_tile.hip
--- a/ntpoly_amd/csrc/spgemm_tile.hip
+++ b/ntpoly_amd/csrc/spgemm_tile.hip
@@ -66,6 +66,21 @@
 constexpr int TILE_DEFER = 48;
 
 
+__device__ inline SlabRun tile_result_run(const double* out_val, int64_t off, int cf, int cl) {
+  const bool any = cl >= cf;
+  const uint64_t addr = reinterpret_cast<uint64_t>(out_val + (any ? off : 0));
+  SlabRun r;
+  r.addr_lo = (uint32_t)addr;
+  r.addr_hi = (uint32_t)(addr >> 32) & 0xffffu;
+  r.nbytes = any ? (uint32_t)(cl - cf + 1) * 8u : 0u;
+  r.flags = kBufferFlags;
+  r.first = any ? cf : (1 << 30);
+  r.first8 = any ? cf * 8 : 0;
+  r.span62 = any ? (cl - cf + 1) + 62 : 0;
+  r.pad = 0;
+  return r;
+}
+
 struct TileArgs {
   const SlabRun* runs;
   const double* bblk;
@@ -77,6 +92,7 @@
   int32_t *ofirst, *olast;
   int64_t* ooff;
   int64_t* otoff;
+  SlabRun* next_runs;
   double alpha, threshold;
   int dense_rule, ncols, nblocks;
   int nrows;
@@ -180,6 +196,7 @@
     a.ooff[a.ncols] = a.blk_toff[a.nblocks];
     if (EPI != 0 && a.otoff) a.otoff[a.nblocks] = a.blk_toff[a.nblocks];
   }
+  if (b == 0 && tid < 4 && a.next_runs) a.next_runs[a.ncols + tid] = tile_result_run(a.out_val, 0, 0, -1);
   if (kn == 0) {
     const int j = b * SLAB_J + tid;
     if (tid < SLAB_J && j < a.ncols) {
@@ -187,6 +204,7 @@
       a.olast[j] = -1;
       a.count[j] = 0;
       a.ooff[j] = tbase + (int64_t)tid * w;
+      if (a.next_runs) a.next_runs[j] = tile_result_run(a.out_val, 0, 0, -1);
       if constexpr (EPI != 0) {
         if (a.fzv.oplast) a.fzv.oplast[j] = -1;
         if (EPI == 2 && a.fzv.xmax[j] >= a.fzv.xmin[j]) atomicOr(a.fzv.flag, 1);
@@ -883,7 +901,9 @@
       a.count[jt] = col_cnt[tid];
       a.ofirst[jt] = cf;
       a.olast[jt] = cl;
-      a.ooff[jt] = tbase + (int64_t)tid * w + (cl >= cf ? cf - lo : 0);
+      const int64_t co = tbase + (int64_t)tid * w + (cl >= cf ? cf - lo : 0);
+      a.ooff[jt] = co;
+      if (a.next_runs) a.next_runs[jt] = tile_result_run(a.out_val, co, cf, cl);
       if constexpr (EPI != 0) {
         if constexpr (LAB) a.fzv.oplast[jt] = col_plast[tid];
       }
@@ -986,7 +1006,7 @@
   a.runs = static_cast<const SlabRun*>(L.runs);
   a.bblk = L.bblk; a.blk_boff = L.blk_boff; a.blk_kmin = L.blk_kmin; a.blk_kn = L.blk_kn; a.blk_lo = L.blk_lo; a.blk_w = L.blk_w;
   a.blk_toff = L.blk_toff; a.out_val = L.out_val; a.count = L.count; a.ofirst = L.ofirst; a.olast = L.olast; a.ooff = L.ooff;
-  a.otoff = L.otoff; a.alpha = L.alpha; a.threshold = L.threshold; a.dense_rule = L.dense_rule; a.ncols = L.ncols;
+  a.otoff = L.otoff; a.next_runs = static_cast<SlabRun*>(L.next_runs); a.alpha = L.alpha; a.threshold = L.threshold; a.dense_rule = L.dense_rule; a.ncols = L.ncols;
   a.nblocks = L.nblocks;
   a.nrows = L.nrows > 0 ? L.nrows : L.ncols;
   a.k4max = std::max(8, (L.max_kn + 3) & ~3);
diff --git a/ntpoly_amd/csrc/spgemm_tile.hpp b/ntpoly_amd/csrc/spgemm_tile.hpp
--- a/ntpoly_amd/csrc/spgemm_tile.hpp
+++ b/ntpoly_amd/csrc/spgemm_tile.hpp
@@ -14,6 +14,7 @@
   int32_t *ofirst = nullptr, *olast = nullptr;
   int64_t* ooff = nullptr;
   int64_t* otoff = nullptr;
+  void* next_runs = nullptr;
   double alpha = 1.0, threshold = 0.0;
   int dense_rule = 0, ncols = 0, nblocks = 0;
   int max_kn = 0, max_w = 0;
diff --git a/ntpoly_amd/csrc/wrp.cpp b/ntpoly_amd/csrc/wrp.cpp
--- a/ntpoly_amd/csrc/wrp.cpp
+++ b/ntpoly_amd/csrc/wrp.cpp
@@ -133,6 +133,7 @@
   else if (n == "increment_force_seq") options().increment_force_seq = *value;
   else if (n == "spgemm_fma") options().spgemm_fma = *value;
   else if (n == "plan_ahead") options().plan_ahead = *value;
+  else if (n == "step_ahead") options().step_ahead = *value;
   else if (n == "slab_algebra") options().slab_algebra = *value;
   else if (n == "operand_cache") options().operand_cache = *value;
   else if (n == "tile_rows") options().tile_rows = *value;
@@ -176,6 +177,7 @@
   if (n == "spgemm_fma") return options().spgemm_fma;
   if (n == "slab_algebra") return options().slab_algebra;
   if (n == "plan_ahead") return options().plan_ahead;
+  if (n == "step_ahead") return options().step_ahead;
   if (n == "tile_rows") return options().tile_rows;
   if (n == "tile2") return options().tile2;
   if (n == "block_path") return options().block_path;
@@ -279,6 +281,9 @@
 }
 void ntpoly_amd_tile2_counts(long long* out) {
   for (int q = 0; q < 2; ++q) out[q] = tile2_counts()[q];
+}
+void ntpoly_amd_step_ahead_counts(long long* out) {
+  for (int q = 0; q < 2; ++q) out[q] = step_ahead_counts()[q];
 }
 void ntpoly_amd_gather_matrix_to_process(const int* ih_this, int* ih_local, const int* within_slice_id) {
   const PSMatrix& m = *get<PSMatrix>(ih_this);
diff --git a/ntpoly_amd/host.py b/ntpoly_amd/host.py
--- a/ntpoly_amd/host.py
+++ b/ntpoly_amd/host.py
@@ -864,6 +864,12 @@
     return dict(done=out[0], repeated=out[1])
 
 
+def step_ahead_counts():
+    out = (C.c_longlong * 2)()
+    lib.ntpoly_amd_step_ahead_counts(out)
+    return dict(prepared=out[0], built=out[1])
+
+
 def band_scope_counts():
     out = (C.c_longlong * 2)()
     lib.ntpoly_amd_band_scope_counts(out)
```

Measured after the change: 694.6, median of 6. 2.3% higher.
